# SeungheonOh/voxtral.c

Hardware: AMD Instinct MI355X
Metric: decoder tokens/sec + encoder RTF, Voxtral-4B bf16 at 1/2/4/8 MI355X (higher is better)
Workload: dtype f32

## Files before the change

include/voxtral_hip.h:

```cpp
#ifndef VOXTRAL_HIP_H
#define VOXTRAL_HIP_H

#include <stddef.h>
#include <stdint.h>

#ifdef __cplusplus
extern "C" {
#endif

int vox_hip_init(void);
int vox_hip_available(void);
void vox_hip_shutdown(void);
size_t vox_hip_memory_used(void);
const char *vox_hip_last_error(void);
void vox_hip_clear_error(void);
int vox_hip_set_device(int device);

typedef struct {
    int enc_dim, enc_layers, enc_heads, enc_kv_heads, enc_head_dim, enc_hidden, enc_window;
    int dec_dim, dec_layers, dec_heads, dec_kv_heads, dec_head_dim, dec_hidden, dec_window;
    int vocab, mel_bins, downsample, ada_dim;
    float rope_theta, enc_eps, dec_eps;
    int gelu_erf;
} vox_hip_config_t;

void vox_hip_config_voxtral_4b(vox_hip_config_t *cfg);

typedef struct {
    const float *conv0_w, *conv0_b, *conv1_w, *conv1_b;
    const uint16_t **enc_wq, **enc_wk, **enc_wv, **enc_wo, **enc_w1, **enc_w2, **enc_w3;
    const float **enc_wq_b, **enc_wv_b, **enc_wo_b, **enc_w2_b, **enc_attn_norm, **enc_ffn_norm;
    const float *enc_norm;
    const uint16_t *ad0, *ad1;
    const uint16_t *tok_emb;
    const uint16_t **dec_wq, **dec_wk, **dec_wv, **dec_wo, **dec_w1, **dec_w2, **dec_w3;
    const float **dec_attn_norm, **dec_ffn_norm, **dec_ada_down, **dec_ada_up;
    const float *dec_norm;
    const float **enc_wq_s, **enc_wk_s, **enc_wv_s, **enc_wo_s, **enc_w1_s, **enc_w2_s, **enc_w3_s;
    const float *ad0_s, *ad1_s, *tok_emb_s;
    const float **dec_wq_s, **dec_wk_s, **dec_wv_s, **dec_wo_s, **dec_w1_s, **dec_w2_s, **dec_w3_s;
} vox_hip_weights_t;

typedef struct vox_hip_model vox_hip_model_t;
typedef struct vox_hip_stream vox_hip_stream_t;

vox_hip_model_t *vox_hip_model_create(const vox_hip_config_t *cfg, const vox_hip_weights_t *w,
                                      int delay_tokens);
void vox_hip_model_free(vox_hip_model_t *m);
int vox_hip_model_set_delay(vox_hip_model_t *m, int delay_tokens);
int vox_hip_model_ada_scale(vox_hip_model_t *m, float *out);
int vox_hip_model_set_kv_fp16(vox_hip_model_t *m, int on);
int vox_hip_set_gemm_planes(int planes);
int vox_hip_gemm_planes(void);
int vox_hip_set_gemmf_wait(int ticks);

vox_hip_stream_t *vox_hip_stream_create(vox_hip_model_t *m);
void vox_hip_stream_free(vox_hip_stream_t *s);
int vox_hip_stream_kv_fp16(const vox_hip_stream_t *s);
int vox_hip_stream_reset(vox_hip_stream_t *s);
int vox_hip_stream_reset_decoder(vox_hip_stream_t *s);

int vox_hip_stream_encode_mel(vox_hip_stream_t *s, const float *mel, int n_frames,
                              int mel_on_device);
int vox_hip_stream_adapter_tokens(vox_hip_stream_t *s);
int vox_hip_stream_set_async_encode(vox_hip_stream_t *s, int on);
int vox_hip_stream_encode_mel_batch(vox_hip_stream_t *const *streams, const float *const *mels,
                                    const int *n_frames, int B, int mel_on_device, int *added);

typedef struct vox_hip_mel vox_hip_mel_t;
vox_hip_mel_t *vox_hip_mel_create(vox_hip_stream_t *s, int left_pad_samples);
int vox_hip_mel_feed(vox_hip_mel_t *m, const float *samples, int n_samples);
int vox_hip_mel_finish(vox_hip_mel_t *m, int right_pad_samples);
int vox_hip_mel_frames(const vox_hip_mel_t *m, int *frame_offset);
const float *vox_hip_mel_frame_ptr(const vox_hip_mel_t *m, int global_frame);
int vox_hip_mel_discard_before(vox_hip_mel_t *m, int keep_from_frame);
int vox_hip_mel_read(vox_hip_mel_t *m, int global_first, int n, float *out);
void vox_hip_mel_free(vox_hip_mel_t *m);
int vox_hip_mel_reset(vox_hip_mel_t *m, int left_pad_samples);
int vox_hip_stream_read_adapter(vox_hip_stream_t *s, int first, int n, float *out);

int vox_hip_stream_decode(vox_hip_stream_t *s, int max_steps, int stop_at_eos,
                          int *tokens_out, float *logits_out);
#define VOX_HIP_MAX_ALT 4
int vox_hip_stream_set_alt(vox_hip_stream_t *s, int n_alt, float cutoff);
int vox_hip_stream_read_alts(vox_hip_stream_t *s, int first, int n, int *ids_out, float *probs_out);
typedef struct vox_hip_batch vox_hip_batch_t;
vox_hip_batch_t *vox_hip_batch_create(vox_hip_model_t *m, int max_streams);
void vox_hip_batch_free(vox_hip_batch_t *b);
int vox_hip_batch_decode(vox_hip_batch_t *b, vox_hip_stream_t **streams, int n, int max_steps,
                         int stop_at_eos, int *tokens_out, int *counts_out);
int vox_hip_batch_decode_rows(vox_hip_batch_t *b, vox_hip_stream_t **streams, int n, const int *rows,
                              int max_steps, int stop_at_eos, int *tokens_out, int *counts_out);
int vox_hip_batch_begin_rows(vox_hip_batch_t *b, vox_hip_stream_t **streams, int n, const int *rows,
                             int max_steps, int stop_at_eos, int *tokens_out, int *counts_out);
int vox_hip_batch_finish(vox_hip_batch_t *b);
int vox_hip_batch_read_logits(vox_hip_batch_t *b, vox_hip_stream_t *s, float *out);
int vox_hip_batch_stats(const vox_hip_batch_t *b, long long *out6);
int vox_hip_stream_state(vox_hip_stream_t *s, int *out6);

void vox_hip_sgemm_bf16(int M, int N, int K, const float *A, const uint16_t *B_bf16, float *C);
void vox_hip_sgemm_q8(int M, int N, int K, const float *A, const int8_t *B_q8, const float *scales,
                      float *C);
void vox_hip_fused_qkv_bf16(int M, int K, const float *input,
                            const uint16_t *wq_bf16, int Nq, const uint16_t *wk_bf16, int Nk,
                            const uint16_t *wv_bf16, int Nv, float *q, float *k, float *v);
void vox_hip_fused_ffn_bf16(int M, int dim, int hidden, const float *input,
                            const uint16_t *w1_bf16, const uint16_t *w3_bf16,
                            const uint16_t *w2_bf16, float *output);
void vox_hip_encoder_attention(float *out, const float *Q, const float *K, const float *V,
                               int seq_q, int seq_k, int n_heads, int n_kv_heads,
                               int head_dim, float scale, int window_size, int q_offset);
int vox_hip_encoder_full_step(vox_hip_stream_t *s, float *x, int new_len,
                              const float *rope_freqs, int logical_start);
int vox_hip_decoder_prefill_step(vox_hip_stream_t *s, float *x, int seq_len,
                                 const float *rope_freqs, int logical_start);
void vox_hip_decoder_start(vox_hip_stream_t *s, const float *x, int dim);
void vox_hip_decoder_end(vox_hip_stream_t *s);
int vox_hip_decoder_full_step(vox_hip_stream_t *s, const float *rope_freqs, int logical_pos,
                              float *logits);

int vox_hip_stream_set_profiling(vox_hip_stream_t *s, int enable);
int vox_hip_stream_profile(vox_hip_stream_t *s, double *out8);
int vox_hip_stream_sync(vox_hip_stream_t *s);

void *vox_hip_device_upload(const void *host, size_t bytes);
int vox_hip_device_free(void *dev);

#ifdef __cplusplus
}
#endif
#endif
```

voxtral.c_amd/csrc/vox_hip.hip:

```cpp
#include "../../include/voxtral_hip.h"
#include "vox_hip_internal.h"

#include <hip/hip_runtime.h>
#include <math.h>
#include <stdarg.h>
#include <stdio.h>
#include <stdlib.h>
#include <string.h>

#include <stddef.h>
#include <algorithm>
#include <atomic>
#include <mutex>
#include <string>
#include <unordered_map>
#include <vector>

using namespace vox;

#define TOKEN_BOS 1
#define TOKEN_EOS 2
#define TOKEN_STREAMING_PAD 32

static thread_local std::string g_err;
static int g_inited = 0;
static size_t g_mem_used = 0;

static int set_err(const char* fmt, ...) {
    char buf[512];
    va_list ap;
    va_start(ap, fmt);
    vsnprintf(buf, sizeof buf, fmt, ap);
    va_end(ap);
    g_err = buf;
    fprintf(stderr, "voxtral_hip: %s\n", buf);
    return -1;
}

#define CK(expr)                                                                          \
    do {                                                                                  \
        hipError_t e__ = (expr);                                                          \
        if (e__ != hipSuccess)                                                            \
            return set_err("%s failed at %s:%d: %s", #expr, __FILE__, __LINE__, hipGetErrorString(e__)); \
    } while (0)

template <class T>
static hipError_t dalloc(T** p, size_t n) {
    *p = nullptr;
    if (n == 0) n = 1;
    hipError_t e = hipMalloc((void**)p, n * sizeof(T));
    if (e == hipSuccess) {
        g_mem_used += n * sizeof(T);
        e = hipMemsetAsync(*p, 0, n * sizeof(T), nullptr);
        if (e == hipSuccess) e = hipStreamSynchronize(nullptr);
    }
    return e;
}
static hipError_t h2d(void* dst, const void* src, size_t bytes) {
    hipError_t e = hipMemcpyAsync(dst, src, bytes, hipMemcpyHostToDevice, nullptr);
    return e == hipSuccess ? hipStreamSynchronize(nullptr) : e;
}
template <class T>
static void dfree(T*& p) {
    if (p) hipFree((void*)p);
    p = nullptr;
}

extern "C" const char* vox_hip_last_error(void) { return g_err.c_str(); }
extern "C" void vox_hip_clear_error(void) { g_err.clear(); }

extern "C" int vox_hip_init(void) {
    int n = 0;
    if (hipGetDeviceCount(&n) != hipSuccess || n <= 0) {
        set_err("no HIP device");
        return 0;
    }
    g_inited = 1;
    return 1;
}
extern "C" int vox_hip_available(void) { return g_inited; }
extern "C" void vox_hip_shutdown(void) { g_inited = 0; }
extern "C" size_t vox_hip_memory_used(void) { return g_mem_used; }
extern "C" int vox_hip_set_device(int device) {
    CK(hipSetDevice(device));
    return 0;
}

extern "C" void vox_hip_config_voxtral_4b(vox_hip_config_t* c) {
    c->enc_dim = 1280; c->enc_layers = 32; c->enc_heads = 32; c->enc_kv_heads = 32;
    c->enc_head_dim = 64; c->enc_hidden = 5120; c->enc_window = 750;
    c->dec_dim = 3072; c->dec_layers = 26; c->dec_heads = 32; c->dec_kv_heads = 8;
    c->dec_head_dim = 128; c->dec_hidden = 9216; c->dec_window = 8192;
    c->vocab = 131072; c->mel_bins = 128; c->downsample = 4; c->ada_dim = 32;
    c->rope_theta = 1000000.0f; c->enc_eps = 1e-5f; c->dec_eps = 1e-5f; c->gelu_erf = 0;
}

static float host_gelu(float v, int erf_mode) {
    if (erf_mode) return 0.5f * v * (1.0f + erff(v * 0.70710678118654752f));
    float x3 = v * v * v;
    float inner = 0.7978845608028654f * (v + 0.044715f * x3);
    return 0.5f * v * (1.0f + tanhf(inner));
}

static void host_rope(float* out, int p0, int n, int dim, float theta) {
    int half = dim / 2;
    for (int s = 0; s < n; s++) {
        float p = (float)(p0 + s);
        for (int d = 0; d < half; d++) {
            float freq = 1.0f / powf(theta, (float)(2 * d) / (float)dim);
            float ang = p * freq;
            out[(size_t)s * dim + 2 * d] = cosf(ang);
            out[(size_t)s * dim + 2 * d + 1] = sinf(ang);
        }
    }
}

struct EncLayerD {
    uint8_t *wqkv, *wo, *w13, *w2;
    float *sqkv, *so, *s13, *s2;
    float *bqkv, *bo, *b2, *attn_norm, *ffn_norm;
};
struct DecLayerD {
    uint8_t *wqkv, *wo, *w13, *w2;
    float *sqkv, *so, *s13, *s2;
    float *attn_norm, *ffn_norm;
};
struct DecFragD {
    uint8_t *wqkv, *wo, *w13, *w2;
};
static int frag_copy(uint8_t** dst, const uint8_t* src, int N, int K, int q8);
struct vox_hip_model;
static int model_frag(vox_hip_model* m);

struct vox_hip_model {
    vox_hip_config_t c;
    int delay_tokens;
    uint16_t *conv0_w, *conv1_w;
    float *conv0_b, *conv1_b, *enc_norm, *dec_norm;
    std::vector<EncLayerD> enc;
    std::vector<DecLayerD> dec;
    uint8_t *ad0, *ad1, *tok_emb;
    float *ad0_s, *ad1_s, *tok_emb_s;
    float* ada_scale;
    std::vector<float> ada_host;
    std::vector<std::vector<float>> ada_down, ada_up;
    float *rope_enc, *rope_dec;
    int rope_positions;
    int rope_gen;
    std::vector<DecFragD> dfrag;
    std::vector<DecFragD> efrag;
    uint8_t* lm_frag;
    int kv16;
};

static int upload(void* dst, const void* src, size_t bytes) {
    if (!src) return set_err("null weight pointer");
    CK(h2d(dst, src, bytes));
    return 0;
}

static int upload_f32_as_bf16(uint16_t* dst, const float* src, size_t n) {
    std::vector<uint16_t> tmp(n);
    for (size_t i = 0; i < n; i++) {
        uint32_t u;
        memcpy(&u, &src[i], 4);
        if (u & 0xffffu) return set_err("conv weight is not bf16-representable (element %zu)", i);
        tmp[i] = (uint16_t)(u >> 16);
    }
    return upload(dst, tmp.data(), n * 2);
}

static int upload_mat(uint8_t** dst, float** dscale, const void* src, const float* scale, size_t rows,
                      size_t cols) {
    const size_t esz = scale ? 1 : 2;
    CK(dalloc(dst, rows * cols * esz));
    if (upload(*dst, src, rows * cols * esz)) return -1;
    *dscale = nullptr;
    if (scale) {
        CK(dalloc(dscale, rows));
        if (upload(*dscale, scale, rows * 4)) return -1;
    }
    return 0;
}

static int upload_qkv(uint8_t** dst, float** dscale, const void* wq, const float* sq, const void* wk,
                      const float* sk, const void* wv, const float* sv, int nq, int nkv, int K) {
    if (!sq != !sk || !sq != !sv) return set_err("wq/wk/wv mix bf16 and Q8");
    const size_t esz = sq ? 1 : 2, rows = (size_t)nq + 2 * nkv;
    CK(dalloc(dst, rows * K * esz));
    if (upload(*dst, wq, (size_t)nq * K * esz) || upload(*dst + (size_t)nq * K * esz, wk, (size_t)nkv * K * esz) ||
        upload(*dst + (size_t)(nq + nkv) * K * esz, wv, (size_t)nkv * K * esz))
        return -1;
    *dscale = nullptr;
    if (sq) {
        CK(dalloc(dscale, rows));
        if (upload(*dscale, sq, (size_t)nq * 4) || upload(*dscale + nq, sk, (size_t)nkv * 4) ||
            upload(*dscale + nq + nkv, sv, (size_t)nkv * 4))
            return -1;
    }
    return 0;
}

static int upload_w13(uint8_t** dst, float** dscale, const void* w1, const float* s1, const void* w3,
                      const float* s3, int hidden, int K) {
    if (!w1 || !w3) return set_err("null w1/w3");
    if (!s1 != !s3) return set_err("w1/w3 mix bf16 and Q8");
    if (hidden % 16) return set_err("hidden %d not a multiple of 16", hidden);
    const size_t esz = s1 ? 1 : 2;
    CK(dalloc(dst, (size_t)2 * hidden * K * esz));
    size_t grp = (size_t)16 * K * esz;
    CK(hipMemcpy2D(*dst, 2 * grp, w1, grp, grp, hidden / 16, hipMemcpyHostToDevice));
    CK(hipMemcpy2D(*dst + grp, 2 * grp, w3, grp, grp, hidden / 16, hipMemcpyHostToDevice));
    *dscale = nullptr;
    if (s1) {
        CK(dalloc(dscale, (size_t)2 * hidden));
        const size_t g4 = 16 * 4;
        CK(hipMemcpy2D(*dscale, 2 * g4, s1, g4, g4, hidden / 16, hipMemcpyHostToDevice));
        CK(hipMemcpy2D((char*)*dscale + g4, 2 * g4, s3, g4, g4, hidden / 16, hipMemcpyHostToDevice));
    }
    return 0;
}

static int model_update_ada(vox_hip_model_t* m) {
    const vox_hip_config_t& c = m->c;
    int D = c.dec_dim, A = c.ada_dim;
    std::vector<float> t_cond(D), hidden(A);
    int half = D / 2;
    float log_theta = logf(10000.0f);
    float t = (float)m->delay_tokens;
    for (int i = 0; i < half; i++) {
        float inv_freq = expf(-log_theta * (float)i / (float)half);
        float emb = t * inv_freq;
        t_cond[i] = cosf(emb);
        t_cond[i + half] = sinf(emb);
    }
    m->ada_host.assign((size_t)c.dec_layers * D, 0.f);
    for (int l = 0; l < c.dec_layers; l++) {
        const float* down = m->ada_down[l].data();
        const float* up = m->ada_up[l].data();
        for (int i = 0; i < A; i++) {
            float sum = 0.f;
            for (int j = 0; j < D; j++) sum += down[(size_t)i * D + j] * t_cond[j];
            hidden[i] = host_gelu(sum, c.gelu_erf);
        }
        float* sc = m->ada_host.data() + (size_t)l * D;
        for (int i = 0; i < D; i++) {
            float sum = 0.f;
            for (int j = 0; j < A; j++) sum += up[(size_t)i * A + j] * hidden[j];
            sc[i] = sum;
        }
    }
    CK(h2d(m->ada_scale, m->ada_host.data(), m->ada_host.size() * 4));
    return 0;
}

static int model_rope_tables(vox_hip_model_t* m, int positions) {
    const vox_hip_config_t& c = m->c;
    dfree(m->rope_enc);
    dfree(m->rope_dec);
    std::vector<float> t((size_t)positions * std::max(c.enc_head_dim, c.dec_head_dim));
    CK(dalloc(&m->rope_enc, (size_t)positions * c.enc_head_dim));
    host_rope(t.data(), 0, positions, c.enc_head_dim, c.rope_theta);
    CK(h2d(m->rope_enc, t.data(), (size_t)positions * c.enc_head_dim * 4));
    CK(dalloc(&m->rope_dec, (size_t)positions * c.dec_head_dim));
    host_rope(t.data(), 0, positions, c.dec_head_dim, c.rope_theta);
    CK(h2d(m->rope_dec, t.data(), (size_t)positions * c.dec_head_dim * 4));
    m->rope_positions = positions;
    m->rope_gen++;
    return 0;
}

static int check_config(const vox_hip_config_t* c) {
    if (c->enc_head_dim != 64 && c->enc_head_dim != 128) return set_err("enc_head_dim must be 64/128");
    if (c->dec_head_dim != 64 && c->dec_head_dim != 128) return set_err("dec_head_dim must be 64/128");
    if (c->enc_heads % c->enc_kv_heads || c->dec_heads % c->dec_kv_heads)
        return set_err("heads must be a multiple of kv heads");
    if (c->dec_heads / c->dec_kv_heads > 4 || c->enc_heads / c->enc_kv_heads > 4)
        return set_err("GQA ratio > 4 unsupported");
    int dims[] = {c->enc_dim, c->enc_hidden, c->dec_dim, c->dec_hidden,
                  c->enc_heads * c->enc_head_dim, c->dec_heads * c->dec_head_dim,
                  c->dec_kv_heads * c->dec_head_dim, c->mel_bins * 3};
    for (int d : dims)
        if (d % 64) return set_err("dimension %d not a multiple of 64", d);
    if (c->vocab % 2) return set_err("vocab must be even");
    if (c->downsample != 4) return set_err("downsample must be 4");
    return 0;
}

extern "C" void vox_hip_model_free(vox_hip_model_t* m);

extern "C" vox_hip_model_t* vox_hip_model_create(const vox_hip_config_t* cfg,
                                                 const vox_hip_weights_t* w, int delay_tokens) {
    if (!g_inited && !vox_hip_init()) return nullptr;
    if (check_config(cfg)) return nullptr;
    vox_hip_model_t* m = new vox_hip_model_t();
    memset(&m->c, 0, sizeof m->c);
    m->c = *cfg;
    m->delay_tokens = delay_tokens;
    {
        const char* e = getenv("VOX_DECODER_KV_FP16");
        m->kv16 = (e && atoi(e) != 0 && cfg->dec_head_dim == 128) ? 1 : 0;
    }
    m->conv0_w = m->conv1_w = nullptr;
    m->ad0 = m->ad1 = m->tok_emb = nullptr;
    m->ad0_s = m->ad1_s = m->tok_emb_s = nullptr;
    m->conv0_b = m->conv1_b = m->enc_norm = m->dec_norm = m->ada_scale = nullptr;
    m->rope_enc = m->rope_dec = nullptr;
    const vox_hip_config_t& c = *cfg;
    const int ED = c.enc_dim, EQ = c.enc_heads * c.enc_head_dim, EKV = c.enc_kv_heads * c.enc_head_dim;
    const int EH = c.enc_hidden;
    const int DD = c.dec_dim, DQ = c.dec_heads * c.dec_head_dim, DKV = c.dec_kv_heads * c.dec_head_dim;
    const int DH = c.dec_hidden;
    auto fail = [&]() -> vox_hip_model_t* { vox_hip_model_free(m); return nullptr; };
#define TRY(x) do { if ((x) != 0) return fail(); } while (0)
#define TRYH(x) do { hipError_t e__ = (x); if (e__ != hipSuccess) { set_err("%s: %s", #x, hipGetErrorString(e__)); return fail(); } } while (0)
#define SCL(field, l) (w->field ? w->field[l] : nullptr)
    TRYH(dalloc(&m->conv0_w, (size_t)ED * c.mel_bins * 3));
    TRY(upload_f32_as_bf16(m->conv0_w, w->conv0_w, (size_t)ED * c.mel_bins * 3));
    TRYH(dalloc(&m->conv1_w, (size_t)ED * ED * 3));
    TRY(upload_f32_as_bf16(m->conv1_w, w->conv1_w, (size_t)ED * ED * 3));
    TRYH(dalloc(&m->conv0_b, ED));
    TRY(upload(m->conv0_b, w->conv0_b, ED * 4));
    TRYH(dalloc(&m->conv1_b, ED));
    TRY(upload(m->conv1_b, w->conv1_b, ED * 4));
    m->enc.resize(c.enc_layers);
    for (int l = 0; l < c.enc_layers; l++) {
        EncLayerD& L = m->enc[l];
        memset(&L, 0, sizeof L);
        TRY(upload_qkv(&L.wqkv, &L.sqkv, w->enc_wq[l], SCL(enc_wq_s, l), w->enc_wk[l], SCL(enc_wk_s, l),
                       w->enc_wv[l], SCL(enc_wv_s, l), EQ, EKV, ED));
        TRYH(dalloc(&L.bqkv, EQ + 2 * EKV));
        TRY(upload(L.bqkv, w->enc_wq_b[l], EQ * 4));
        TRY(upload(L.bqkv + EQ + EKV, w->enc_wv_b[l], EKV * 4));
        TRY(upload_mat(&L.wo, &L.so, w->enc_wo[l], SCL(enc_wo_s, l), ED, EQ));
        TRYH(dalloc(&L.bo, ED));
        TRY(upload(L.bo, w->enc_wo_b[l], ED * 4));
        TRY(upload_w13(&L.w13, &L.s13, w->enc_w1[l], SCL(enc_w1_s, l), w->enc_w3[l], SCL(enc_w3_s, l), EH, ED));
        TRY(upload_mat(&L.w2, &L.s2, w->enc_w2[l], SCL(enc_w2_s, l), ED, EH));
        TRYH(dalloc(&L.b2, ED));
        TRY(upload(L.b2, w->enc_w2_b[l], ED * 4));
        TRYH(dalloc(&L.attn_norm, ED));
        TRY(upload(L.attn_norm, w->enc_attn_norm[l], ED * 4));
        TRYH(dalloc(&L.ffn_norm, ED));
        TRY(upload(L.ffn_norm, w->enc_ffn_norm[l], ED * 4));
    }
    TRYH(dalloc(&m->enc_norm, ED));
    TRY(upload(m->enc_norm, w->enc_norm, ED * 4));
    TRY(upload_mat(&m->ad0, &m->ad0_s, w->ad0, w->ad0_s, DD, (size_t)ED * c.downsample));
    TRY(upload_mat(&m->ad1, &m->ad1_s, w->ad1, w->ad1_s, DD, DD));
    TRY(upload_mat(&m->tok_emb, &m->tok_emb_s, w->tok_emb, w->tok_emb_s, c.vocab, DD));
    m->dec.resize(c.dec_layers);
    m->ada_down.resize(c.dec_layers);
    m->ada_up.resize(c.dec_layers);
    for (int l = 0; l < c.dec_layers; l++) {
        DecLayerD& L = m->dec[l];
        memset(&L, 0, sizeof L);
        TRY(upload_qkv(&L.wqkv, &L.sqkv, w->dec_wq[l], SCL(dec_wq_s, l), w->dec_wk[l], SCL(dec_wk_s, l),
                       w->dec_wv[l], SCL(dec_wv_s, l), DQ, DKV, DD));
        TRY(upload_mat(&L.wo, &L.so, w->dec_wo[l], SCL(dec_wo_s, l), DD, DQ));
        TRY(upload_w13(&L.w13, &L.s13, w->dec_w1[l], SCL(dec_w1_s, l), w->dec_w3[l], SCL(dec_w3_s, l), DH, DD));
        TRY(upload_mat(&L.w2, &L.s2, w->dec_w2[l], SCL(dec_w2_s, l), DD, DH));
        TRYH(dalloc(&L.attn_norm, DD));
        TRY(upload(L.attn_norm, w->dec_attn_norm[l], DD * 4));
        TRYH(dalloc(&L.ffn_norm, DD));
        TRY(upload(L.ffn_norm, w->dec_ffn_norm[l], DD * 4));
        if (!w->dec_ada_down[l] || !w->dec_ada_up[l]) { set_err("null ada weights"); return fail(); }
        m->ada_down[l].assign(w->dec_ada_down[l], w->dec_ada_down[l] + (size_t)c.ada_dim * DD);
        m->ada_up[l].assign(w->dec_ada_up[l], w->dec_ada_up[l] + (size_t)DD * c.ada_dim);
    }
    TRYH(dalloc(&m->dec_norm, DD));
    TRY(upload(m->dec_norm, w->dec_norm, DD * 4));
    TRYH(dalloc(&m->ada_scale, (size_t)c.dec_layers * DD));
    TRY(model_update_ada(m));
    TRY(model_rope_tables(m, 32768));
#undef TRY
#undef TRYH
#undef SCL
    return m;
}

extern "C" void vox_hip_model_free(vox_hip_model_t* m) {
    if (!m) return;
    dfree(m->conv0_w); dfree(m->conv1_w); dfree(m->conv0_b); dfree(m->conv1_b);
    for (auto& L : m->enc) {
        dfree(L.wqkv); dfree(L.wo); dfree(L.w13); dfree(L.w2);
        dfree(L.sqkv); dfree(L.so); dfree(L.s13); dfree(L.s2);
        dfree(L.bqkv); dfree(L.bo); dfree(L.b2); dfree(L.attn_norm); dfree(L.ffn_norm);
    }
    for (auto& L : m->dec) {
        dfree(L.wqkv); dfree(L.wo); dfree(L.w13); dfree(L.w2);
        dfree(L.sqkv); dfree(L.so); dfree(L.s13); dfree(L.s2);
        dfree(L.attn_norm); dfree(L.ffn_norm);
    }
    for (auto& F : m->dfrag) {
        dfree(F.wqkv); dfree(F.wo); dfree(F.w13); dfree(F.w2);
    }
    for (auto& F : m->efrag) {
        dfree(F.wqkv); dfree(F.wo); dfree(F.w13); dfree(F.w2);
    }
    dfree(m->lm_frag);
    dfree(m->enc_norm); dfree(m->ad0); dfree(m->ad1); dfree(m->tok_emb); dfree(m->dec_norm);
    dfree(m->ad0_s); dfree(m->ad1_s); dfree(m->tok_emb_s);
    dfree(m->ada_scale); dfree(m->rope_enc); dfree(m->rope_dec);
    delete m;
}

extern "C" int vox_hip_model_set_delay(vox_hip_model_t* m, int delay_tokens) {
    m->delay_tokens = delay_tokens;
    return model_update_ada(m);
}

extern "C" int vox_hip_set_gemm_planes(int planes) {
    if (set_gemm_planes(planes)) return set_err("gemm planes: 2 or 3 (got %d)", planes);
    return 0;
}

extern "C" int vox_hip_gemm_planes(void) { return gemm_planes_np(); }
extern "C" int vox_hip_set_gemmf_wait(int ticks) { return set_gemmf_wait(ticks); }

extern "C" int vox_hip_model_set_kv_fp16(vox_hip_model_t* m, int on) {
    if (on && m->c.dec_head_dim != 128) return set_err("16-bit decoder KV: head_dim 128 only (got %d)", m->c.dec_head_dim);
    m->kv16 = on ? 1 : 0;
    return 0;
}

extern "C" int vox_hip_stream_kv_fp16(const vox_hip_stream_t* s);

extern "C" int vox_hip_model_ada_scale(vox_hip_model_t* m, float* out) {
    memcpy(out, m->ada_host.data(), m->ada_host.size() * 4);
    return 0;
}

static const int ENC_SUB = 1024;
static const int DEC_SLACK = 64;
static const int STEP_BATCH = 16;
static const size_t GEMM_WS_ELEMS = (size_t)8 << 20;
static const int TOKENS_CAP = 1 << 16;

struct vox_hip_stream {
    vox_hip_stream() { memset((void*)this, 0, offsetof(vox_hip_stream, pev)); }
    vox_hip_model_t* m;
    unsigned long long uid;
    hipStream_t st;
    float *ek, *ev, *dk, *dv;
    int ecap, dcap;
    int kv16;
    long long enc_pos;
    float *mel_p, *mel_tail, *c0_p, *c0_tail, *c0_res, *im2col;
    int res_count;
    int frames_cap;
    float *x_enc, *xn, *qkv, *q, *att, *gate, *enc_res;
    int x_rows_cap;
    int enc_res_count;
    float *rope_rows;
    int rope_rows_cap;
    float *adapter, *ad_mid;
    int adapter_cap, total_adapter;
    float *xd, *xnd, *qkvd, *qd_, *attd, *gated, *part, *logits, *pval;
    float *part_alt, *alts;
    float* gws;
    size_t gws_n;
    uint16_t* exp_;
    float* eslab;
    uint16_t* exp2;
    int* eticket;
    int enc_async;
    float* xbatch;
    float *cs_im, *cs_c0;
    float *abatch, *abatch_out;
    float* essq;
    uint16_t *gpa, *gpc;
    int* gflags;
    int gepoch;
    uint16_t *dpa, *dpc;
    int dp_rows;
    int n_alt;
    float alt_cutoff;
    int graph_alt;
    int graph_rope_gen;
    int *pidx, *state, *tokens;
    int* twin_state;
    int dec_rows_cap, tokens_cap;
    hipGraphExec_t step_exec[STEP_GRAPHS];
    int graph_ready;
    int started, eos_seen, n_generated;
    int h_state[4];
    int profiling;
    int graph_prof;
    int capturing;
    hipEvent_t evt[2];
    hipEvent_t sev;
    std::vector<hipEvent_t> pev;
    double prof_ms, prof_bytes;
    long long prof_launches;
};

static int stream_alloc_frames(vox_hip_stream_t* s, int frames) {
    if (frames <= s->frames_cap) return 0;
    const vox_hip_config_t& c = s->m->c;
    int f = 256;
    while (f < frames) f *= 2;
    dfree(s->mel_p); dfree(s->c0_p); dfree(s->im2col); dfree(s->x_enc);
    CK(dalloc(&s->mel_p, (size_t)(f + 2) * c.mel_bins));
    CK(dalloc(&s->c0_p, (size_t)(f + 3) * c.enc_dim));
    size_t im = std::max((size_t)f * c.mel_bins * 3, (size_t)(f / 2 + 2) * c.enc_dim * 3);
    CK(dalloc(&s->im2col, im));
    CK(dalloc(&s->x_enc, (size_t)(f / 2 + 8) * c.enc_dim));
    s->frames_cap = f;
    return 0;
}

static int stream_alloc_adapter(vox_hip_stream_t* s, int need) {
    if (need <= s->adapter_cap) return 0;
    const int D = s->m->c.dec_dim;
    int nc = s->adapter_cap ? s->adapter_cap : 1024;
    while (nc < need) nc *= 2;
    float* na = nullptr;
    CK(dalloc(&na, (size_t)nc * D));
    if (s->adapter && s->total_adapter > 0)
        CK(hipMemcpyAsync(na, s->adapter, (size_t)s->total_adapter * D * 4, hipMemcpyDeviceToDevice, s->st));
    CK(hipStreamSynchronize(s->st));
    dfree(s->adapter);
    s->adapter = na;
    s->adapter_cap = nc;
    s->graph_ready = 0;
    return 0;
}

static int stream_alloc_dec_rows(vox_hip_stream_t* s, int rows) {
    if (rows <= s->dec_rows_cap) return 0;
    const vox_hip_config_t& c = s->m->c;
    int r = 64;
    while (r < rows) r *= 2;
    const int DQ = c.dec_heads * c.dec_head_dim, DKV = c.dec_kv_heads * c.dec_head_dim;
    dfree(s->xd); dfree(s->xnd); dfree(s->qkvd); dfree(s->qd_); dfree(s->attd); dfree(s->gated);
    CK(dalloc(&s->xd, (size_t)r * c.dec_dim));
    CK(dalloc(&s->xnd, (size_t)r * c.dec_dim));
    CK(dalloc(&s->qkvd, (size_t)r * (DQ + 2 * DKV)));
    CK(dalloc(&s->qd_, (size_t)r * DQ));
    CK(dalloc(&s->attd, (size_t)r * DQ));
    CK(dalloc(&s->gated, (size_t)r * c.dec_hidden));
    s->dec_rows_cap = r;
    s->graph_ready = 0;
    return 0;
}

extern "C" void vox_hip_stream_free(vox_hip_stream_t* s);

extern "C" vox_hip_stream_t* vox_hip_stream_create(vox_hip_model_t* m) {
    static std::atomic<unsigned long long> next_uid{1};
    vox_hip_stream_t* s = new vox_hip_stream_t();
    s->m = m;
    s->uid = next_uid++;
    const vox_hip_config_t& c = m->c;
    auto fail = [&]() -> vox_hip_stream_t* { vox_hip_stream_free(s); return nullptr; };
#define TRYH(x) do { hipError_t e__ = (x); if (e__ != hipSuccess) { set_err("%s: %s", #x, hipGetErrorString(e__)); return fail(); } } while (0)
#define SCL(field, l) (w->field ? w->field[l] : nullptr)
// ... 1017 lines not shown
    }
    if (!s->enc_async) CK(hipStreamSynchronize(s->st));
    return added;
}

extern "C" int vox_hip_stream_set_async_encode(vox_hip_stream_t* s, int on) {
    if (!s) return set_err("null stream");
    if (s->enc_async && !on) CK(hipStreamSynchronize(s->st));
    s->enc_async = on ? 1 : 0;
    return 0;
}

extern "C" int vox_hip_stream_adapter_tokens(vox_hip_stream_t* s) { return s->total_adapter; }

extern "C" int vox_hip_stream_read_adapter(vox_hip_stream_t* s, int first, int n, float* out) {
    const int D = s->m->c.dec_dim;
    if (first < 0 || first + n > s->total_adapter) return set_err("adapter rows out of range");
    CK(hipMemcpyAsync(out, s->adapter + (size_t)first * D, (size_t)n * D * 4, hipMemcpyDeviceToHost, s->st));
    CK(hipStreamSynchronize(s->st));
    return 0;
}

static int stream_prefilled(vox_hip_stream_t* s, hipStream_t q) {
    const int np = 32 + s->m->delay_tokens;
    const int st4[4] = {np, np, TOKEN_STREAMING_PAD, s->n_generated};
    CK(hipMemcpyAsync(s->state, st4, sizeof st4, hipMemcpyHostToDevice, q));
    s->h_state[0] = np;
    s->h_state[1] = np;
    s->h_state[2] = TOKEN_STREAMING_PAD;
    s->h_state[3] = s->n_generated;
    s->started = 1;
    return 0;
}

static int dec_gemmf_env() {
    static int v = -1;
    if (v < 0) {
        const char* e = getenv("VOX_HIP_PREFILL_GEMMF");
        v = (e && atoi(e) == 0) ? 0 : 1;
    }
    return v;
}

static bool dec_gemmf_ok(const vox_hip_model_t* m, int n) {
    const vox_hip_config_t& c = m->c;
    const int DD = c.dec_dim, DQ = c.dec_heads * c.dec_head_dim, DKV = c.dec_kv_heads * c.dec_head_dim;
    return enc_gemmf_env() && dec_gemmf_env() && !m->dec[0].sqkv && n >= 1 && n <= PLANE_MAX_ROWS && gemmf_ok(n, DQ + 2 * DKV, DD) &&
           gemmf_ok(n, DD, DQ) && gemmf_ok(n, 2 * c.dec_hidden, DD) && gemmf_ok(n, DD, c.dec_hidden) &&
           c.dec_hidden % 64 == 0;
}

static int stream_dec_planes(vox_hip_stream_t* s, int rows) {
    if (rows <= s->dp_rows) return 0;
    const vox_hip_config_t& c = s->m->c;
    const int DD = c.dec_dim, DQ = c.dec_heads * c.dec_head_dim;
    const int r = (rows + 127) / 128 * 128;
    dfree(s->dpa);
    dfree(s->dpc);
    s->dp_rows = 0;
    CK(dalloc(&s->dpa, (size_t)r * 3 * std::max(DD, DQ)));
    CK(dalloc(&s->dpc, (size_t)r * 3 * c.dec_hidden));
    if (!s->gflags) CK(dalloc(&s->gflags, gemmf_flag_ints()));
    s->dp_rows = r;
    return 0;
}

template <class Attn>
static int dec_layers_gemmf(vox_hip_stream_t* s, const GemmfQ& q, float* x, int n, Attn attn) {
    vox_hip_model_t* m = s->m;
    const vox_hip_config_t& c = m->c;
    const int DD = c.dec_dim, DQ = c.dec_heads * c.dec_head_dim, DKV = c.dec_kv_heads * c.dec_head_dim;
    const int DH = c.dec_hidden;
    if (model_frag(m) || stream_dec_planes(s, n)) return -1;
    for (int l = 0; l < c.dec_layers; l++) {
        const DecLayerD& L = m->dec[l];
        const DecFragD& F = m->dfrag[l];
        CK(launch_rmsnorm_fplanes(x, n, DD, L.attn_norm, nullptr, c.dec_eps, s->dpa, nullptr, 0, q.st));
        if (gemmf_on(q, EPI_STORE, s->dpa, DD, n, F.wqkv, DQ + 2 * DKV, nullptr, s->qkvd, DQ + 2 * DKV, nullptr)) return -1;
        if (attn(l)) return -1;
        if (gemmf_on(q, EPI_RESID, s->dpa, DQ, n, F.wo, DD, nullptr, x, DD, nullptr)) return -1;
        CK(launch_rmsnorm_fplanes(x, n, DD, L.ffn_norm, m->ada_scale + (size_t)l * DD, c.dec_eps, s->dpa, nullptr, 0,
                                  q.st));
        if (gemmf_on(q, EPI_SWIGLU, s->dpa, DD, n, F.w13, 2 * DH, nullptr, nullptr, DH, s->dpc)) return -1;
        if (gemmf_on(q, EPI_RESID, s->dpc, DH, n, F.w2, DD, nullptr, x, DD, nullptr)) return -1;
    }
    return 0;
}

static int run_decoder_rows(vox_hip_stream_t* s, float* x, int n, int pos0, const float* rope) {
    vox_hip_model_t* m = s->m;
    const vox_hip_config_t& c = m->c;
    const int DD = c.dec_dim, H = c.dec_heads, KVH = c.dec_kv_heads, hd = c.dec_head_dim;
    const int DQ = H * hd, DKV = KVH * hd, DH = c.dec_hidden;
    const float scale = 1.0f / sqrtf((float)hd);
    hipStream_t st = s->st;
    if (stream_alloc_dec_rows(s, n)) return -1;
    if (n > DEC_SLACK + 1 && pos0 > 0) return set_err("prefill of %d rows on a non-empty cache", n);
    bool gf = n > 1 && dec_gemmf_ok(m, n);
    if (gf && (model_frag(m) || stream_dec_planes(s, n))) {
        vox_hip_clear_error();
        (void)hipGetLastError();
        gf = false;
    }
    if (gf) {
        if (!s->gflags) CK(dalloc(&s->gflags, gemmf_flag_ints()));
        return dec_layers_gemmf(s, GemmfQ{st, s->gws, s->gws_n, s->gflags, &s->gepoch}, x, n, [&](int l) -> int {
            float* Kc = dec_ring(s, s->dk, l);
            float* Vc = dec_ring(s, s->dv, l);
            CK(launch_rope_kv(s->qkvd, n, DQ, DKV, hd, rope, pos0, s->qd_, Kc, Vc, s->dcap, st, s->kv16));
            CK(launch_attn_rows_mf(hd, s->qd_, DQ, Kc, Vc, s->dcap, s->attd, DQ, n, H, KVH, pos0, 0, c.dec_window, scale,
                                   st, s->gws, s->gws_n, s->dpa, s->kv16));
            return 0;
        });
    }
    for (int l = 0; l < c.dec_layers; l++) {
        const DecLayerD& L = m->dec[l];
        float* Kc = dec_ring(s, s->dk, l);
        float* Vc = dec_ring(s, s->dv, l);
        CK(launch_rmsnorm_rows(x, DD, s->xnd, DD, L.attn_norm, nullptr, n, DD, c.dec_eps, st));
        CK(launch_gemm(EPI_STORE, 3, s->xnd, DD, L.wqkv, L.sqkv, DD, n, DQ + 2 * DKV, nullptr, s->qkvd, DQ + 2 * DKV, st, s->gws, s->gws_n));
        CK(launch_rope_kv(s->qkvd, n, DQ, DKV, hd, rope, pos0, s->qd_, Kc, Vc, s->dcap, st, s->kv16));
        CK(launch_attn_rows_mf(hd, s->qd_, DQ, Kc, Vc, s->dcap, s->attd, DQ, n, H, KVH, pos0, 0, c.dec_window, scale, st,
                             s->gws, s->gws_n, nullptr, s->kv16));
        CK(launch_gemm(EPI_RESID, 3, s->attd, DQ, L.wo, L.so, DQ, n, DD, nullptr, x, DD, st, s->gws, s->gws_n));
        CK(launch_rmsnorm_rows(x, DD, s->xnd, DD, L.ffn_norm, m->ada_scale + (size_t)l * DD, n, DD, c.dec_eps, st));
        CK(launch_gemm(EPI_SWIGLU, 3, s->xnd, DD, L.w13, L.s13, DD, n, 2 * DH, nullptr, s->gated, DH, st, s->gws, s->gws_n));
        CK(launch_gemm(EPI_RESID, 3, s->gated, DH, L.w2, L.s2, DH, n, DD, nullptr, x, DD, st, s->gws, s->gws_n));
    }
    return 0;
}

static int enqueue_lm_head(vox_hip_stream_t* s, const int* state);

static int enqueue_step_layers(vox_hip_stream_t* s, const int* state, int pos, const float* rope_row,
                               int splits) {
    vox_hip_model_t* m = s->m;
    const vox_hip_config_t& c = m->c;
    const int DD = c.dec_dim, H = c.dec_heads, KVH = c.dec_kv_heads, hd = c.dec_head_dim;
    const int DQ = H * hd, DKV = KVH * hd, DH = c.dec_hidden;
    const float scale = 1.0f / sqrtf((float)hd);
    hipStream_t st = s->st;
    for (int l = 0; l < c.dec_layers; l++) {
        const DecLayerD& L = m->dec[l];
        float* Kc = dec_ring(s, s->dk, l);
        float* Vc = dec_ring(s, s->dv, l);
        GemvArgs a;
        memset(&a, 0, sizeof a);
        a.x = s->xd; a.K = DD; a.W = L.wqkv; a.wscale = L.sqkv; a.rows = DQ + 2 * DKV;
        a.norm_w = L.attn_norm; a.eps = c.dec_eps; a.y = s->qd_;
        a.qd = DQ; a.kvd = DKV; a.hd = hd;
        a.state = state; a.pos = pos;
        a.rope = state ? m->rope_dec : rope_row - (size_t)pos * hd;
        a.Kc = Kc; a.Vc = Vc; a.cap = s->dcap; a.kv16 = s->kv16;
        CK(launch_gemv(PRO_NORM, EPI_QKV, a, st));
        CK(launch_attn_decode(hd, s->qd_, Kc, Vc, s->dcap, state, pos, c.dec_window, scale, H, KVH,
                              s->part, s->attd, splits, st, s->kv16));
        memset(&a, 0, sizeof a);
        a.x = s->attd; a.K = DQ; a.W = L.wo; a.wscale = L.so; a.rows = DD; a.y = s->xd;
        CK(launch_gemv(PRO_NONE, EPI_RESID, a, st));
        memset(&a, 0, sizeof a);
        a.x = s->xd; a.K = DD; a.W = L.w13; a.wscale = L.s13; a.rows = 2 * DH; a.norm_w = L.ffn_norm;
        a.ada = m->ada_scale + (size_t)l * DD; a.eps = c.dec_eps; a.y = s->gated;
        const bool gprof = s->profiling && state && !s->capturing && (int)s->pev.size() == 2 * c.dec_layers;
        if (gprof) CK(launch_gemv_timed(PRO_NORM_ADA, EPI_SWIGLU, a, s->pev[2 * l], s->pev[2 * l + 1], st));
        else CK(launch_gemv(PRO_NORM_ADA, EPI_SWIGLU, a, st));
        memset(&a, 0, sizeof a);
        a.x = s->gated; a.K = DH; a.W = L.w2; a.wscale = L.s2; a.rows = DD; a.y = s->xd;
        CK(launch_gemv(PRO_NONE, EPI_RESID, a, st));
    }
    return enqueue_lm_head(s, state);
}

static int enqueue_lm_head(vox_hip_stream_t* s, const int* state) {
    vox_hip_model_t* m = s->m;
    const vox_hip_config_t& c = m->c;
    hipStream_t st = s->st;
    GemvArgs a;
    memset(&a, 0, sizeof a);
    a.x = s->xd; a.K = c.dec_dim; a.W = m->tok_emb; a.wscale = m->tok_emb_s; a.rows = c.vocab; a.norm_w = m->dec_norm;
    a.eps = c.dec_eps; a.y = s->logits; a.part_val = s->pval; a.part_idx = s->pidx;
    a.part_alt = s->part_alt;
    CK(launch_gemv(PRO_NORM, (state && s->n_alt > 1) ? EPI_LOGITS_ALT : EPI_LOGITS, a, st));
    return 0;
}

static int graph_splits(const vox_hip_stream_t* s, int g) {
    return std::min(1 << g, attn_maxsplits(s->m->c.dec_window));
}

static int graph_index(const vox_hip_stream_t* s, int ctx) {
    const int need = (ctx + ATT_BLOCK_KEYS - 1) / ATT_BLOCK_KEYS;
    int g = 0;
    while ((1 << g) < need && (1 << g) < attn_maxsplits(s->m->c.dec_window)) g++;
    return g;
}

static int enqueue_graph_step(vox_hip_stream_t* s, int splits) {
    const vox_hip_config_t& c = s->m->c;
    if (enqueue_step_layers(s, s->state, 0, nullptr, splits)) return -1;
    CK(launch_argmax_final(s->pval, s->pidx, gemv_grid(c.vocab), s->state, s->tokens, s->tokens_cap,
                           s->adapter, s->adapter_cap, s->m->tok_emb, s->m->tok_emb_s, c.dec_dim, s->xd,
                           s->part_alt, s->n_alt > 1 ? s->alts : nullptr, s->st));
    return 0;
}

static int build_step_graph(vox_hip_stream_t* s, int gi) {
    if (s->step_exec[gi]) {
        hipGraphExecDestroy(s->step_exec[gi]);
        s->step_exec[gi] = nullptr;
    }
    hipGraph_t g = nullptr;
    CK(hipStreamBeginCapture(s->st, hipStreamCaptureModeThreadLocal));
    s->capturing = 1;
    int rc = enqueue_graph_step(s, graph_splits(s, gi));
    s->capturing = 0;
    hipError_t e = hipStreamEndCapture(s->st, &g);
    if (rc || e != hipSuccess) {
        if (g) hipGraphDestroy(g);
        return set_err("graph capture failed: %s", hipGetErrorString(e));
    }
    e = hipGraphInstantiate(&s->step_exec[gi], g, nullptr, nullptr, 0);
    hipGraphDestroy(g);
    if (e != hipSuccess) return set_err("graph instantiate failed: %s", hipGetErrorString(e));
    s->graph_ready |= 1 << gi;
    s->graph_alt = s->n_alt > 1;
    s->graph_rope_gen = s->m->rope_gen;
    return 0;
}

static int collect_graph_profile(vox_hip_stream_t* s) {
    if (!s->profiling || !s->graph_prof) return 0;
    const vox_hip_config_t& c = s->m->c;
    for (int l = 0; l < c.dec_layers; l++) {
        float ms = 0.f;
        CK(hipEventElapsedTime(&ms, s->pev[2 * l], s->pev[2 * l + 1]));
        s->prof_ms += ms;
        s->prof_bytes += (double)2 * c.dec_hidden * c.dec_dim * 2;
        s->prof_launches++;
    }
    return 0;
}

static int use_graphs() {
    static int v = -1;
    if (v < 0) {
        const char* e = getenv("VOX_HIP_GRAPH");
        v = (e && atoi(e) == 0) ? 0 : 1;
    }
    return v;
}

static int run_steps(vox_hip_stream_t* s, int n, int pos0) {
    const vox_hip_config_t& c = s->m->c;
    const int gi = graph_index(s, std::min(pos0 + n, c.dec_window));
    const int splits = graph_splits(s, gi);
    if (s->profiling && use_graphs() && n > 1) {
        s->profiling = 0;
        const int rc = run_steps(s, n - 1, pos0);
        s->profiling = 1;
        if (rc) return -1;
        pos0 += n - 1;
        n = 1;
    }
    if (!use_graphs() || s->profiling) {
        if (s->profiling && s->pev.empty()) {
            s->pev.resize(2 * c.dec_layers);
            for (auto& e : s->pev) CK(hipEventCreate(&e));
        }
        s->graph_prof = s->profiling;
        for (int i = 0; i < n; i++)
            if (enqueue_graph_step(s, splits)) return -1;
        return 0;
    }
    if (s->graph_ready && (s->graph_alt != (s->n_alt > 1) || s->graph_rope_gen != s->m->rope_gen)) s->graph_ready = 0;
    if (!(s->graph_ready & (1 << gi)) && build_step_graph(s, gi)) return -1;
    for (int i = 0; i < n; i++) CK(hipGraphLaunch(s->step_exec[gi], s->st));
    return 0;
}

template <class T>
static int ring_read(const T* ring, int cap, int rec, long long first, int n, T* out, hipStream_t st) {
    while (n > 0) {
        const int slot = (int)(first % cap);
        const int k = std::min(n, cap - slot);
        CK(hipMemcpyAsync(out, ring + (size_t)slot * rec, (size_t)k * rec * sizeof(T), hipMemcpyDeviceToHost, st));
        out += (size_t)k * rec;
        first += k;
        n -= k;
    }
    return 0;
}

static int stream_prefill(vox_hip_stream_t* s) {
    vox_hip_model_t* m = s->m;
    const int np = 32 + m->delay_tokens;
    if (stream_alloc_dec_rows(s, np)) return -1;
    if (ensure_rope(s, np + 2)) return -1;
    CK(launch_embed_rows(s->adapter, m->tok_emb, m->tok_emb_s, 0, np, TOKEN_BOS, TOKEN_STREAMING_PAD, m->c.dec_dim,
                         s->xd, s->st));
    if (run_decoder_rows(s, s->xd, np, 0, m->rope_dec)) return -1;
    return stream_prefilled(s, s->st);
}

extern "C" int vox_hip_stream_decode(vox_hip_stream_t* s, int max_steps, int stop_at_eos,
                                     int* tokens_out, float* logits_out) {
    vox_hip_model_t* m = s->m;
    const vox_hip_config_t& c = m->c;
    const int D = c.dec_dim, V = c.vocab, hd = c.dec_head_dim;
    const int prompt_len = 1 + 32 + m->delay_tokens;
    int produced = 0;
    if (max_steps <= 0 || s->eos_seen) return 0;
    if (!s->started) {
        if (s->total_adapter < prompt_len) return 0;
        if (stream_prefill(s)) return -1;
    }
    const int step_base = s->n_generated;
    int avail = s->total_adapter - (s->h_state[1] > 0 ? s->h_state[1] : prompt_len - 1);
    {
        int st4[4];
        CK(hipMemcpyAsync(st4, s->state, sizeof st4, hipMemcpyDeviceToHost, s->st));
        CK(hipStreamSynchronize(s->st));
        memcpy(s->h_state, st4, sizeof st4);
        avail = s->total_adapter - st4[1];
    }
    if (ensure_rope(s, (long long)s->h_state[0] + avail + 1)) return -1;
    if (avail > 0) CK(launch_embed_step(s->adapter, m->tok_emb, m->tok_emb_s, s->state, D, s->xd, s->st));
    int todo = std::min(max_steps, avail);
    std::vector<int> tok;
    while (produced < todo) {
        int b = std::min(STEP_BATCH, todo - produced);
        if (logits_out) b = 1;
        if (run_steps(s, b, s->h_state[0] + produced)) return -1;
        tok.resize(produced + b);
        if (ring_read(s->tokens, s->tokens_cap, 1, (long long)step_base + produced, b, tok.data() + produced, s->st))
// ... 69 lines not shown
            if (pr) pr[k] = p;
        }
    }
    return 0;
}

extern "C" int vox_hip_stream_state(vox_hip_stream_t* s, int* out6) {
    out6[0] = s->h_state[0];
    out6[1] = s->h_state[1];
    out6[2] = s->h_state[2];
    out6[3] = s->started;
    out6[4] = s->eos_seen;
    out6[5] = s->n_generated;
    return 0;
}

extern "C" int vox_hip_stream_set_profiling(vox_hip_stream_t* s, int enable) {
    s->profiling = enable;
    s->prof_ms = 0;
    s->prof_bytes = 0;
    s->prof_launches = 0;
    return 0;
}

extern "C" int vox_hip_stream_profile(vox_hip_stream_t* s, double* out8) {
    out8[0] = s->prof_ms;
    out8[1] = s->prof_bytes;
    out8[2] = (double)s->prof_launches;
    out8[3] = s->prof_launches ? s->prof_ms / s->prof_launches : 0.0;
    out8[4] = 0;
    out8[5] = s->prof_launches ? s->prof_bytes / s->prof_launches : 0.0;
    int rec = 0;
    if (s->gflags) {
        CK(hipMemcpyAsync(&rec, s->gflags + gemmf_grid(), sizeof rec, hipMemcpyDeviceToHost, s->st));
        CK(hipStreamSynchronize(s->st));
    }
    out8[6] = rec;
    out8[7] = 0.0;
    return 0;
}

struct TwinW {
    uint8_t* w;
    float* s;
    int N, K, Np, Kp;
};
struct TwinKey {
    const void* p;
    int n, k;
    bool operator==(const TwinKey& o) const { return p == o.p && n == o.n && k == o.k; }
};
struct TwinKeyHash {
    size_t operator()(const TwinKey& t) const {
        return std::hash<const void*>()(t.p) ^ ((size_t)t.n * 0x9e3779b97f4a7c15ull) ^ ((size_t)t.k << 1);
    }
};
static std::mutex g_twin_mu;
static std::unordered_map<TwinKey, TwinW, TwinKeyHash> g_wcache;
static hipStream_t g_twin_st = nullptr;
static float* g_twin_ws = nullptr;
static float *g_tA = nullptr, *g_tC = nullptr, *g_tQ = nullptr, *g_tK = nullptr, *g_tV = nullptr, *g_tO = nullptr;
static size_t g_tA_n = 0, g_tC_n = 0, g_tQ_n = 0, g_tK_n = 0, g_tV_n = 0, g_tO_n = 0;
static float* g_tWs = nullptr;
static size_t g_tWs_n = 0;

static int pad_to(int v, int a) { return (v + a - 1) / a * a; }

static int twin_buf(float** p, size_t* cap, size_t n) {
    if (n <= *cap) return 0;
    dfree(*p);
    *cap = 0;
    CK(dalloc(p, n));
    *cap = n;
    return 0;
}

static const TwinW* twin_weight(const void* host, const float* scales, int N, int K) {
    if (!host || N <= 0 || K <= 0) {
        set_err("twin weight: null pointer or empty shape (%d x %d)", N, K);
        return nullptr;
    }
    const TwinKey key{host, N, K};
    auto it = g_wcache.find(key);
    if (it != g_wcache.end()) return &it->second;
    TwinW t{nullptr, nullptr, N, K, pad_to(N, 128), pad_to(K, 64)};
    const size_t esz = scales ? 1 : 2;
    hipError_t e = dalloc(&t.w, (size_t)t.Np * t.Kp * esz);
    if (e == hipSuccess)
        e = hipMemcpy2DAsync(t.w, (size_t)t.Kp * esz, host, (size_t)K * esz, (size_t)K * esz, N,
                             hipMemcpyHostToDevice, g_twin_st);
    if (e == hipSuccess && scales) {
        e = dalloc(&t.s, (size_t)t.Np);
        if (e == hipSuccess) e = hipMemcpyAsync(t.s, scales, (size_t)N * 4, hipMemcpyHostToDevice, g_twin_st);
    }
    if (e == hipSuccess) e = hipStreamSynchronize(g_twin_st);
    if (e != hipSuccess) {
        dfree(t.w);
        dfree(t.s);
        set_err("twin weight upload (%d x %d): %s", N, K, hipGetErrorString(e));
        return nullptr;
    }
    return &(g_wcache[key] = t);
}

static int twin_init() {
    if (!g_inited && !vox_hip_init()) return -1;
    if (!g_twin_st) CK(hipStreamCreateWithFlags(&g_twin_st, hipStreamNonBlocking));
    if (!g_twin_ws) CK(dalloc(&g_twin_ws, GEMM_WS_ELEMS));
    return 0;
}

static int twin_put_rows(float** buf, size_t* cap, const float* host, int M, int K, int Kp) {
    if (!host) return set_err("twin: null input");
    if (twin_buf(buf, cap, (size_t)M * Kp)) return -1;
    if (Kp != K) {
        CK(hipMemsetAsync(*buf, 0, (size_t)M * Kp * 4, g_twin_st));
        CK(hipMemcpy2DAsync(*buf, (size_t)Kp * 4, host, (size_t)K * 4, (size_t)K * 4, M, hipMemcpyHostToDevice,
                            g_twin_st));
    } else {
        CK(hipMemcpyAsync(*buf, host, (size_t)M * K * 4, hipMemcpyHostToDevice, g_twin_st));
    }
    return 0;
}

static int twin_get_rows(float* host, const float* dev, int M, int N, int Np) {
    if (!host) return set_err("twin: null output");
    CK(hipMemcpy2DAsync(host, (size_t)N * 4, dev, (size_t)Np * 4, (size_t)N * 4, M, hipMemcpyDeviceToHost, g_twin_st));
    return 0;
}

static int twin_gemm_dev(int M, const float* dA, const TwinW& W, float* dC) {
    if (M == 1 && gemv_ok(W.Np, W.Kp, W.s != nullptr)) {
        GemvArgs a;
        memset(&a, 0, sizeof a);
        a.x = dA; a.K = W.Kp; a.W = W.w; a.wscale = W.s; a.rows = W.Np; a.y = dC;
        CK(launch_gemv(PRO_NONE, EPI_STORE, a, g_twin_st));
        return 0;
    }
    CK(launch_gemm(EPI_STORE, 3, dA, W.Kp, W.w, W.s, W.Kp, M, W.Np, nullptr, dC, W.Np, g_twin_st, g_twin_ws,
                   GEMM_WS_ELEMS));
    return 0;
}

static int twin_sgemm(int M, int N, int K, const float* A, const void* B, const float* scales, float* C) {
    if (M <= 0 || N <= 0 || K <= 0) return M == 0 ? 0 : set_err("sgemm: bad shape %d x %d x %d", M, N, K);
    if (twin_init()) return -1;
    const TwinW* W = twin_weight(B, scales, N, K);
    if (!W) return -1;
    if (twin_put_rows(&g_tA, &g_tA_n, A, M, K, W->Kp) || twin_buf(&g_tC, &g_tC_n, (size_t)M * W->Np) ||
        twin_gemm_dev(M, g_tA, *W, g_tC) || twin_get_rows(C, g_tC, M, N, W->Np))
        return -1;
    CK(hipStreamSynchronize(g_twin_st));
    return 0;
}

extern "C" void vox_hip_sgemm_bf16(int M, int N, int K, const float* A, const uint16_t* B, float* C) {
    std::lock_guard<std::mutex> lk(g_twin_mu);
    twin_sgemm(M, N, K, A, B, nullptr, C);
}

extern "C" void vox_hip_sgemm_q8(int M, int N, int K, const float* A, const int8_t* B, const float* scales,
                                 float* C) {
    std::lock_guard<std::mutex> lk(g_twin_mu);
    if (!scales) { set_err("sgemm_q8: null scales"); return; }
    twin_sgemm(M, N, K, A, B, scales, C);
}

extern "C" void vox_hip_fused_qkv_bf16(int M, int K, const float* input, const uint16_t* wq, int Nq,
                                       const uint16_t* wk, int Nk, const uint16_t* wv, int Nv,
                                       float* q, float* k, float* v) {
    std::lock_guard<std::mutex> lk(g_twin_mu);
    if (M <= 0) return;
    if (twin_init()) return;
    const TwinW* W[3] = {twin_weight(wq, nullptr, Nq, K), twin_weight(wk, nullptr, Nk, K),
                         twin_weight(wv, nullptr, Nv, K)};
    if (!W[0] || !W[1] || !W[2]) return;
    float* outs[3] = {q, k, v};
    float* dO[3] = {nullptr, nullptr, nullptr};
    size_t* caps[3] = {&g_tQ_n, &g_tK_n, &g_tV_n};
    float** bufs[3] = {&g_tQ, &g_tK, &g_tV};
    if (twin_put_rows(&g_tA, &g_tA_n, input, M, K, W[0]->Kp)) return;
    for (int i = 0; i < 3; i++) {
        if (twin_buf(bufs[i], caps[i], (size_t)M * W[i]->Np) || twin_gemm_dev(M, g_tA, *W[i], *bufs[i])) return;
        dO[i] = *bufs[i];
    }
    for (int i = 0; i < 3; i++)
        if (twin_get_rows(outs[i], dO[i], M, W[i]->N, W[i]->Np)) return;
    if (hipStreamSynchronize(g_twin_st) != hipSuccess) set_err("fused_qkv: sync failed");
}

__global__ void k_silu_mul(float* g, const float* u, size_t n) {
    size_t i = (size_t)blockIdx.x * 256 + threadIdx.x;
    if (i < n) {
        float v = g[i];
        g[i] = v / (1.0f + expf(-v)) * u[i];
    }
}

extern "C" void vox_hip_fused_ffn_bf16(int M, int dim, int hidden, const float* input,
                                       const uint16_t* w1, const uint16_t* w3, const uint16_t* w2,
                                       float* output) {
    std::lock_guard<std::mutex> lk(g_twin_mu);
    if (M <= 0) return;
    if (twin_init()) return;
    const TwinW* d1 = twin_weight(w1, nullptr, hidden, dim);
    const TwinW* d3 = twin_weight(w3, nullptr, hidden, dim);
    const TwinW* d2 = twin_weight(w2, nullptr, dim, hidden);
    if (!d1 || !d3 || !d2) return;
    const int Hp = d1->Np;
    if (d2->Kp != Hp) { set_err("fused_ffn: padded hidden %d != %d", d2->Kp, Hp); return; }
    if (twin_put_rows(&g_tA, &g_tA_n, input, M, dim, d1->Kp) || twin_buf(&g_tQ, &g_tQ_n, (size_t)M * Hp) ||
        twin_buf(&g_tK, &g_tK_n, (size_t)M * Hp) || twin_buf(&g_tC, &g_tC_n, (size_t)M * d2->Np) ||
        twin_gemm_dev(M, g_tA, *d1, g_tQ) || twin_gemm_dev(M, g_tA, *d3, g_tK))
        return;
    const size_t n = (size_t)M * Hp;
    hipLaunchKernelGGL(k_silu_mul, dim3((unsigned)((n + 255) / 256)), dim3(256), 0, g_twin_st, g_tQ, g_tK, n);
    if (hipGetLastError() != hipSuccess) { set_err("fused_ffn: silu_mul launch failed"); return; }
    if (twin_gemm_dev(M, g_tQ, *d2, g_tC) || twin_get_rows(output, g_tC, M, dim, d2->Np)) return;
    if (hipStreamSynchronize(g_twin_st) != hipSuccess) set_err("fused_ffn: sync failed");
}

static int twin_attention(float* out, const float* Q, const float* K, const float* V, int seq_q, int seq_k,
                          int n_heads, int n_kv_heads, int head_dim, float scale, int window_size, int q_offset) {
    if (twin_init()) return -1;
    if (seq_q <= 0) return 0;
    if (!out || !Q || !K || !V) return set_err("encoder_attention: null pointer");
    if (q_offset < 0 || q_offset + seq_q > seq_k) return set_err("encoder_attention: queries beyond keys");
    if (n_kv_heads <= 0 || n_heads % n_kv_heads) return set_err("encoder_attention: heads %d / kv heads %d", n_heads, n_kv_heads);
    const size_t qn = (size_t)seq_q * n_heads * head_dim, kn = (size_t)seq_k * n_kv_heads * head_dim;
    if (twin_buf(&g_tQ, &g_tQ_n, qn) || twin_buf(&g_tK, &g_tK_n, kn) || twin_buf(&g_tV, &g_tV_n, kn) ||
        twin_buf(&g_tO, &g_tO_n, qn))
        return -1;
    CK(hipMemcpyAsync(g_tQ, Q, qn * 4, hipMemcpyHostToDevice, g_twin_st));
    CK(hipMemcpyAsync(g_tK, K, kn * 4, hipMemcpyHostToDevice, g_twin_st));
    CK(hipMemcpyAsync(g_tV, V, kn * 4, hipMemcpyHostToDevice, g_twin_st));
    const int W = window_size > 0 ? window_size : (1 << 30);
    float* ws = nullptr;
    size_t wsn = 0;
    if (n_heads * ((seq_q + 15) / 16) < 256) {
        wsn = (size_t)n_heads * seq_q * 16 * (head_dim + 2);
        if (twin_buf(&g_tWs, &g_tWs_n, wsn)) return -1;
        ws = g_tWs;
    }
    CK(launch_attn_rows_mf(head_dim, g_tQ, n_heads * head_dim, g_tK, g_tV, seq_k, g_tO, n_heads * head_dim, seq_q,
                         n_heads, n_kv_heads, q_offset, 0, W, scale, g_twin_st, ws, wsn));
    CK(hipMemcpyAsync(out, g_tO, qn * 4, hipMemcpyDeviceToHost, g_twin_st));
    CK(hipStreamSynchronize(g_twin_st));
    return 0;
}

extern "C" void vox_hip_encoder_attention(float* out, const float* Q, const float* K, const float* V,
                                          int seq_q, int seq_k, int n_heads, int n_kv_heads,
                                          int head_dim, float scale, int window_size, int q_offset) {
    std::lock_guard<std::mutex> lk(g_twin_mu);
    twin_attention(out, Q, K, V, seq_q, seq_k, n_heads, n_kv_heads, head_dim, scale, window_size, q_offset);
}

static int upload_rope_rows(vox_hip_stream_t* s, const float* rope, size_t n) {
    if (n > (size_t)s->rope_rows_cap) {
        dfree(s->rope_rows);
        CK(dalloc(&s->rope_rows, n));
        s->rope_rows_cap = (int)n;
    }
    CK(hipMemcpyAsync(s->rope_rows, rope, n * 4, hipMemcpyHostToDevice, s->st));
    return 0;
}

extern "C" int vox_hip_encoder_full_step(vox_hip_stream_t* s, float* x, int new_len,
                                         const float* rope_freqs, int logical_start) {
    const vox_hip_config_t& c = s->m->c;
    const int ED = c.enc_dim;
    if (stream_alloc_frames(s, 2 * new_len + 8)) return -1;
    float* xin = s->x_enc + (size_t)4 * ED;
    CK(hipMemcpyAsync(xin, x, (size_t)new_len * ED * 4, hipMemcpyHostToDevice, s->st));
    if (upload_rope_rows(s, rope_freqs, (size_t)new_len * c.enc_head_dim)) return -1;
    for (int r0 = 0; r0 < new_len; r0 += ENC_SUB) {
        int nr = std::min(ENC_SUB, new_len - r0);
        if (run_encoder_rows(s, xin + (size_t)r0 * ED, nr, (long long)logical_start + r0,
                             s->rope_rows + (size_t)r0 * c.enc_head_dim))
            return -1;
    }
    CK(hipMemcpyAsync(x, xin, (size_t)new_len * ED * 4, hipMemcpyDeviceToHost, s->st));
    CK(hipStreamSynchronize(s->st));
    return 0;
}

extern "C" int vox_hip_decoder_prefill_step(vox_hip_stream_t* s, float* x, int seq_len,
                                            const float* rope_freqs, int logical_start) {
    const vox_hip_config_t& c = s->m->c;
    if (stream_alloc_dec_rows(s, seq_len)) return -1;
    CK(hipMemcpyAsync(s->xd, x, (size_t)seq_len * c.dec_dim * 4, hipMemcpyHostToDevice, s->st));
    if (upload_rope_rows(s, rope_freqs, (size_t)seq_len * c.dec_head_dim)) return -1;
    if (run_decoder_rows(s, s->xd, seq_len, logical_start, s->rope_rows)) return -1;
    CK(hipMemcpyAsync(x, s->xd, (size_t)seq_len * c.dec_dim * 4, hipMemcpyDeviceToHost, s->st));
    CK(hipStreamSynchronize(s->st));
    return 0;
}

extern "C" void vox_hip_decoder_start(vox_hip_stream_t* s, const float* x, int dim) {
    if (!s || !x || dim != s->m->c.dec_dim) {
        set_err("decoder_start: dim %d != dec_dim", dim);
        return;
    }
    if (hipMemcpyAsync(s->xd, x, (size_t)dim * 4, hipMemcpyHostToDevice, s->st) != hipSuccess)
        set_err("decoder_start upload failed");
}
// ... 590 lines not shown
```

voxtral.c_amd/csrc/vox_hip_dev.h:

```cpp
#pragma once
#include <hip/hip_runtime.h>
#include <stdint.h>

#include "vox_hip_internal.h"

namespace vox {

typedef __attribute__((ext_vector_type(8))) __bf16 bf16x8;
typedef __attribute__((ext_vector_type(4))) float f32x4;
typedef __attribute__((ext_vector_type(2))) float f32x2;
typedef __attribute__((ext_vector_type(4))) unsigned int u32x4;
typedef __attribute__((ext_vector_type(2))) unsigned int u32x2;

__device__ __forceinline__ uint4 ldnt(const uint4* p) {
    u32x4 v = __builtin_nontemporal_load(reinterpret_cast<const u32x4*>(p));
    return make_uint4(v.x, v.y, v.z, v.w);
}

__device__ __forceinline__ float bf2f(uint32_t bits16) { return __uint_as_float(bits16 << 16); }
__device__ __forceinline__ float bflo(uint32_t w) { return __uint_as_float(w << 16); }
__device__ __forceinline__ float bfhi(uint32_t w) { return __uint_as_float(w & 0xffff0000u); }

__device__ __forceinline__ uint32_t f2bf(float f) {
    const __bf16 b = (__bf16)f;
    return __builtin_bit_cast(unsigned short, b);
}

template <int CTRL>
__device__ __forceinline__ float dpp(float v) {
    return __int_as_float(__builtin_amdgcn_update_dpp(0, __float_as_int(v), CTRL, 0xF, 0xF, false));
}
__device__ __forceinline__ float rows4_sum(float v) {
    const int iv = __float_as_int(v);
    const float a = __int_as_float(__builtin_amdgcn_readlane(iv, 0)), b = __int_as_float(__builtin_amdgcn_readlane(iv, 16));
    const float c = __int_as_float(__builtin_amdgcn_readlane(iv, 32)), d = __int_as_float(__builtin_amdgcn_readlane(iv, 48));
    return (a + b) + (c + d);
}
__device__ __forceinline__ float rows4_max(float v) {
    const int iv = __float_as_int(v);
    const float a = __int_as_float(__builtin_amdgcn_readlane(iv, 0)), b = __int_as_float(__builtin_amdgcn_readlane(iv, 16));
    const float c = __int_as_float(__builtin_amdgcn_readlane(iv, 32)), d = __int_as_float(__builtin_amdgcn_readlane(iv, 48));
    return fmaxf(fmaxf(a, b), fmaxf(c, d));
}
__device__ __forceinline__ float row_sum16(float v) {
    v += dpp<0xB1>(v);
    v += dpp<0x4E>(v);
    v += dpp<0x141>(v);
    v += dpp<0x140>(v);
    return v;
}
__device__ __forceinline__ float row_max16(float v) {
    v = fmaxf(v, dpp<0xB1>(v));
    v = fmaxf(v, dpp<0x4E>(v));
    v = fmaxf(v, dpp<0x141>(v));
    v = fmaxf(v, dpp<0x140>(v));
    return v;
}
__device__ __forceinline__ float wave_sum(float v) {
    v = row_sum16(v);
    v += __shfl_xor(v, 16, 64);
    v += __shfl_xor(v, 32, 64);
    return v;
}
__device__ __forceinline__ float wave_sum63(float v) {
    v = row_sum16(v);
    v += __int_as_float(__builtin_amdgcn_update_dpp(0, __float_as_int(v), 0x142, 0xA, 0xF, false));
    v += __int_as_float(__builtin_amdgcn_update_dpp(0, __float_as_int(v), 0x143, 0xC, 0xF, false));
    return v;
}
__device__ __forceinline__ float wave_max(float v) {
    v = row_max16(v);
    v = fmaxf(v, __shfl_xor(v, 16, 64));
    v = fmaxf(v, __shfl_xor(v, 32, 64));
    return v;
}

__device__ __forceinline__ float gelu_tanh(float v) {
    float x3 = v * v * v;
    float inner = 0.7978845608028654f * (v + 0.044715f * x3);
    return 0.5f * v * (1.0f + tanhf(inner));
}
__device__ __forceinline__ float gelu_erf(float v) { return 0.5f * v * (1.0f + erff(v * 0.70710678118654752f)); }
__device__ __forceinline__ float silu(float v) { return v / (1.0f + expf(-v)); }

__device__ __forceinline__ void split3(float v, uint16_t& h, uint16_t& m, uint16_t& l) {
    const uint32_t b0 = f2bf(v);
    const float r1 = v - __uint_as_float(b0 << 16);
    const uint32_t b1 = f2bf(r1);
    const float r2 = r1 - __uint_as_float(b1 << 16);
    h = (uint16_t)b0;
    m = (uint16_t)b1;
    l = (uint16_t)f2bf(r2);
}

__device__ __forceinline__ size_t frag_off(int j, int k) {
    const int b = k >> 6, r = k & 63;
    return ((size_t)(b * 2 + ((r >> 3) & 1)) * 64 + (r >> 4) * 16 + j) * 8 + (r & 7);
}

__device__ __forceinline__ float psum(const float* __restrict__ part, int S, int N, int j, int n) {
    part += (size_t)(j >> 4) * S * SK_ROWS * N;
    j &= 15;
    float v = part[(size_t)j * N + n];
#pragma unroll 4
    for (int s = 1; s < S; s++) v += part[((size_t)s * SK_ROWS + j) * N + n];
    return v;
}
__device__ __forceinline__ float2 psum2(const float* __restrict__ part, int S, int N, int j, int n) {
    part += (size_t)(j >> 4) * S * SK_ROWS * N + (size_t)(j & 15) * N + n;
    const size_t stride = (size_t)SK_ROWS * N;
    float2 v = *reinterpret_cast<const float2*>(part);
    for (int s0 = 1; s0 < S; s0 += 8) {
        float2 t[8];
#pragma unroll
        for (int c = 0; c < 8; c++)
            t[c] = s0 + c < S ? *reinterpret_cast<const float2*>(part + (s0 + c) * stride) : make_float2(0.f, 0.f);
#pragma unroll
        for (int c = 0; c < 8; c++)
            if (s0 + c < S) {
                v.x += t[c].x;
                v.y += t[c].y;
            }
    }
    return v;
}
__device__ __forceinline__ size_t frag_at(int j, int K, int p, int k) {
    return ((size_t)(j >> 4) * 3 + p) * SK_ROWS * K + frag_off(j & 15, k);
}

__device__ __forceinline__ float dot8(uint4 w, float4 a, float4 b, float acc) {
    acc = fmaf(bflo(w.x), a.x, acc);
    acc = fmaf(bfhi(w.x), a.y, acc);
    acc = fmaf(bflo(w.y), a.z, acc);
    acc = fmaf(bfhi(w.y), a.w, acc);
    acc = fmaf(bflo(w.z), b.x, acc);
    acc = fmaf(bfhi(w.z), b.y, acc);
    acc = fmaf(bflo(w.w), b.z, acc);
    acc = fmaf(bfhi(w.w), b.w, acc);
    return acc;
}

__device__ __forceinline__ float i8f(uint32_t w, int b) { return (float)((int32_t)(w << (24 - 8 * b)) >> 24); }
__device__ __forceinline__ float dot16q(uint4 w, const float4 (&x)[4], float acc) {
    const uint32_t d[4] = {w.x, w.y, w.z, w.w};
#pragma unroll
    for (int k = 0; k < 4; k++) {
        acc = fmaf(i8f(d[k], 0), x[k].x, acc);
        acc = fmaf(i8f(d[k], 1), x[k].y, acc);
        acc = fmaf(i8f(d[k], 2), x[k].z, acc);
        acc = fmaf(i8f(d[k], 3), x[k].w, acc);
    }
    return acc;
}

}
```

voxtral.c_amd/csrc/vox_hip_internal.h:

```cpp
#pragma once
#include <hip/hip_runtime.h>
#include <stdint.h>

namespace vox {

enum { EPI_STORE = 0, EPI_RESID = 1, EPI_GELU = 2, EPI_GELU_ERF = 3, EPI_SWIGLU = 4, EPI_QKV = 5, EPI_LOGITS = 6,
       EPI_LOGITS_ALT = 7,
       EPI_PARTIAL = 8,
       EPI_QKV_BIAS = 9 };
constexpr int ALT_TEXT_MIN = 1000;
constexpr int ALT_PART = 10;
constexpr int ALT_REC = 8;
enum { PRO_NONE = 0, PRO_NORM = 1, PRO_NORM_ADA = 2 };

constexpr int GEMV_MAX_BLOCKS = 1024;

struct GemvArgs {
    const float* x;
    int K;
    const void* W;
    const float* wscale;
    int rows;
    const float* norm_w;
    const float* ada;
    float eps;
    float* y;
    const float* bias;
    int qd, kvd, hd;
    const float* rope;
    const int* state;
    int pos;
    float* Kc;
    float* Vc;
    int cap;
    int kv16 = 0;
    float* part_val;
    int* part_idx;
    float* part_alt;
};

constexpr int VOX_MAX_BATCH = 32;

struct BatchSlot {
    int* state;
    int* tokens;
    const float* adapter;
    char* Kc;
    char* Vc;
    float* alts;
    int adapter_rows;
    int left;
    int stop_tok;
    int live;
    int pos;
    int produced;
};
static_assert(sizeof(BatchSlot) == 72, "BatchSlot layout");
constexpr int BATCH_TOKLOG = 64;

struct AttnPtrs {
    const float* q[VOX_MAX_BATCH];
    const float* Kc[VOX_MAX_BATCH];
    const float* Vc[VOX_MAX_BATCH];
    const int* state[VOX_MAX_BATCH];
    float* part[VOX_MAX_BATCH];
    float* out[VOX_MAX_BATCH];
    const BatchSlot* slots = nullptr;
    size_t ring_off = 0;
};

struct AttnFuse {
    const float* qkv;
    int S, N;
    const float* rope;
    uint16_t* xs;
};

constexpr int ARGB = 64;

int gemv_grid(int rows);
bool gemv_ok(int rows, int K, int q8);
int attn_maxch(int window);
int attn_maxsplits(int window);
hipError_t launch_rmsnorm_rows(const float* x, int ldx, float* y, int ldy, const float* w,
                               const float* ada, int M, int D, float eps, hipStream_t st);
hipError_t launch_gemm(int epi, int nsplit, const float* A, int lda, const void* W,
                       const float* wscale, int K, int M, int N, const float* bias, float* C,
                       int ldc, hipStream_t st, float* ws = nullptr, size_t ws_elems = 0);
hipError_t launch_rope_kv(const float* qkv, int M, int qd, int kvd, int hd, const float* rope,
                          int pos0, float* q, float* Kc, float* Vc, int cap, hipStream_t st, int kv16 = 0);
hipError_t launch_attn_rows_mf(int hd, const float* Q, int ldq, const float* Kc, const float* Vc,
                             int cap, float* O, int ldo, int M, int H, int KVH, int q_pos0,
                             int k_first, int window, float scale, hipStream_t st, float* ws = nullptr,
                             size_t ws_elems = 0, uint16_t* xs = nullptr, int kv16 = 0);
hipError_t launch_slabs_rope_kv(const float* part, int S, int M, const float* bias, int qd, int kvd, int hd,
                                const float* rope, int pos0, float* q, float* Kc, float* Vc, int cap, hipStream_t st);
hipError_t launch_gemv(int pro, int epi, const GemvArgs& a, hipStream_t st);
const void* gemv_kernel(int pro, int epi, const GemvArgs& a);
hipError_t launch_gemv_timed(int pro, int epi, const GemvArgs& a, hipEvent_t start, hipEvent_t stop,
                             hipStream_t st);
int gemv_occupancy(const void* fn);
hipError_t launch_attn_decode(int hd, const float* q, const float* Kc, const float* Vc, int cap,
                              const int* state, int pos_host, int window, float scale, int H,
                              int KVH, float* part, float* out, int splits, hipStream_t st, int kv16 = 0);
hipError_t launch_attn_decode_batch(int hd, const AttnPtrs& p, int nb, int cap, int window, float scale,
                                    int H, int KVH, int splits, hipStream_t st, int kv16 = 0);
constexpr int ATT_BLOCK_KEYS = 256;
hipError_t launch_attn_batch_fused(int hd, const AttnPtrs& p, const AttnFuse& f, int nb, int cap, int window,
                                   float scale, int H, int KVH, int splits, hipStream_t st, int kv16 = 0);

struct EncRows {
    int B;
    int off[VOX_MAX_BATCH], nr[VOX_MAX_BATCH], pos0[VOX_MAX_BATCH];
    float* Kc[VOX_MAX_BATCH];
    float* Vc[VOX_MAX_BATCH];
};
hipError_t launch_rope_kv_rows(const float* qkv, int N, int qd, int kvd, int hd, const float* rope_table,
                               const EncRows& er, float* q, int cap, hipStream_t st);
hipError_t launch_attn_rows(int hd, const float* Q, const EncRows& er, int N, int cap, float* O, int H, int KVH,
                            int window, float scale, float* ws, size_t ws_elems, hipStream_t st, uint16_t* xs = nullptr);
constexpr int STEP_GRAPHS = 8;
hipError_t launch_attn_batch_dbg(const AttnPtrs& p, const AttnFuse& f, int nb, int cap, int window, float scale, int H,
                                 int KVH, int splits, hipStream_t st);
hipError_t launch_attn_dbg(int dbg, const float* q, const float* Kc, const float* Vc, int cap,
                           const int* state, float* part, float* out, hipStream_t st);
hipError_t launch_embed_step(const float* adapter, const void* emb, const float* esc, const int* state,
                             int D, float* x, hipStream_t st);
hipError_t launch_embed_rows(const float* adapter, const void* emb, const float* esc, int row0, int n,
                             int first_tok, int rest_tok, int D, float* x, hipStream_t st);
hipError_t launch_argmax_final(const float* pv, const int* pi, int n, int* state, int* tokens,
                               int cap, const float* adapter, int adapter_rows,
                               const void* emb, const float* esc, int D, float* x,
                               const float* part_alt, float* alts, hipStream_t st);
hipError_t launch_embed_batch(const BatchSlot* slots, int nb, const void* emb, const float* esc, int D, float* x,
                              hipStream_t st);
hipError_t launch_argmax_batch(const float* logits, int nb, int V, float* pval, int* pidx, float* palt,
                               BatchSlot* slots, int tokens_cap, int* toklog, const void* emb, const float* esc, int D,
                               float* x, hipStream_t st);
#ifdef VOX_KBENCH
#define VOX_KB_KNOB(name, v) int name = v
#else
#define VOX_KB_KNOB(name, v) constexpr int name = v
#endif
constexpr int SK_ROWS = 16;
constexpr int SK_MAX_ROWS = 96;
constexpr int PLANE_MAX_ROWS = 1024;
hipError_t launch_frag_pack(const void* src, int N, int K, int q8, void* dst, hipStream_t st);
hipError_t launch_rmsnorm_fplanes(float* x, int nb, int D, const float* w, const float* ada, float eps,
                                  uint16_t* xs, const float* part, int S, hipStream_t st, const float* bias = nullptr);
hipError_t launch_resid_slabs(float* x, int nb, int D, const float* part, int S, const float* bias, hipStream_t st);
hipError_t launch_slabs_rows(const float* part, int S, int nb, int N, const float* bias, float* out, int ldo,
                             hipStream_t st);
hipError_t launch_split_fplanes(const float* x, int nb, int K, uint16_t* xs, hipStream_t st);
hipError_t launch_swiglu_fplanes(const float* part, int S, int H, int nb, uint16_t* xs, hipStream_t st);
hipError_t launch_gemm_skf(const uint16_t* xs, int K, const void* Wf, const float* wscale, int N, int nb, float* C,
                           int ldc, hipStream_t st);
hipError_t launch_gemm_skf2(const uint16_t* xs, int K, const void* Wf, const float* wscale, int N, int nb, float* C,
                            int ldc, hipStream_t st);
int skl_splits(int K, int N = 0);
constexpr int SKL_MAX_SLICES = 12;
hipError_t launch_gemm_skl(const uint16_t* xs, int K, const void* Wf, const float* wscale, int N, int nb,
                           float* part, hipStream_t st, const float* ssq = nullptr, int nsl = 0, float eps = 0.f,
                           int pair = 0);
hipError_t launch_gemm_skl_cfg(int nw, int ks, const uint16_t* xs, int K, const void* Wf, int N, int nb, float* part,
                               hipStream_t st);
hipError_t launch_gemm_skl2_cfg(int nw, int ks, const uint16_t* xs, int K, const void* Wf, int N, int nb, float* part,
                                hipStream_t st);
hipError_t launch_resid_xw_fplanes(float* x, int nb, int D, const float* w, const float* ada, uint16_t* xs,
                                   const float* part, int S, const float* bias, float* ssq, hipStream_t st);
enum { SKX_PRO_PLANES = 0, SKX_PRO_SCALE = 1 };
enum { SKX_EPI_QKV = 1, SKX_EPI_RESID = 2, SKX_EPI_SWIGLU = 3 };
struct SklFused {
    const float* ssq_in = nullptr;
    int nsl = 0;
    float eps = 0.f;
    float* part = nullptr;
    int* ticket = nullptr;
    const float* bias = nullptr;
    float* x = nullptr;
    float* ssq_out = nullptr;
    uint16_t* planes = nullptr;
    const float* nw = nullptr;
    const float* ada = nullptr;
    const float* rope = nullptr;
    int qd = 0, kvd = 0, hd = 0, pos0 = 0, cap = 0;
    float* q = nullptr;
    float* Kc = nullptr;
    float* Vc = nullptr;
};
int sklx_slices(int N, int K);
constexpr int SKX_TICKETS = 4 * 1024;
hipError_t launch_gemm_sklx(int pro, int epi, const uint16_t* xs, int K, const void* Wf, int N, int nb,
                            const SklFused& f, hipStream_t st);
bool gemmf_ok(int M, int N, int K);
int gemmf_grid();
size_t gemmf_flag_ints();
int set_gemmf_wait(int ticks);
size_t gemmf_ws_floats(int blocks);
hipError_t launch_gemmf(int epi, int np, const uint16_t* xs, int K, int M, const void* Wf, int N, const float* bias,
                        float* C, int ldc, uint16_t* xo, float* ws, size_t ws_floats, int* flags, int epoch,
                        hipStream_t st);
int gemm_planes_np();
int set_gemm_planes(int np);
hipError_t launch_im2col3(const float* src, int C, int T, int stride, int off, float* A,
                          hipStream_t st);
hipError_t launch_mel_tail(const float* melp, int n_new, int MB, float* tail, hipStream_t st);
hipError_t launch_mel_frames(const float* samples, long long start0, int nframes, const float* window,
                             const float* dcosT, const float* dsinT, const float* filtT, float log_min, float* mel,
                             hipStream_t st);
hipError_t launch_mel_reflect(float* buf, long long n, long long real_end, int len, hipStream_t st);

}
```

voxtral.c_amd/csrc/vox_hip_kernels.hip:

```cpp
#include "vox_hip_internal.h"
#include "vox_hip_dev.h"

#include <hip/hip_runtime.h>
#include <hip/hip_ext.h>
#include <stdint.h>
#include <algorithm>
#include <string.h>
#include <stdlib.h>

namespace vox {

typedef _Float16 kvh_t;
typedef _Float16 h16x4 __attribute__((ext_vector_type(4)));
typedef _Float16 h16x2 __attribute__((ext_vector_type(2)));
template <class T> __device__ __forceinline__ float4 kv_ld4(const T* p) {
    if constexpr (sizeof(T) == 4) {
        return *reinterpret_cast<const float4*>(p);
    } else {
        const h16x4 h = *reinterpret_cast<const h16x4*>(p);
        return make_float4((float)h[0], (float)h[1], (float)h[2], (float)h[3]);
    }
}
template <class T> __device__ __forceinline__ float2 kv_ld2(const T* p) {
    if constexpr (sizeof(T) == 4) {
// ... 453 lines not shown
                for (int b = 0; b < NB; b++) vv[c][b] = vn[c][b];
        }
    }
    if (g == 0) {
        sm[wave][j] = m;
        sl[wave][j] = l;
    }
#pragma unroll
    for (int i = 0; i < 4; i++)
#pragma unroll
        for (int b = 0; b < NB; b++) so[wave][4 * g + i][NB * j + b] = acc[b][i];
    __syncthreads();
    const int r = tid >> 4, d0 = (tid & 15) * NB;
    if (r >= nq) return;
    float mx = -1e30f;
#pragma unroll
    for (int w = 0; w < 4; w++) mx = fmaxf(mx, sm[w][r]);
    float f[4], den = 0.f;
#pragma unroll
    for (int w = 0; w < 4; w++) {
        f[w] = expf(sm[w][r] - mx);
        den = fmaf(f[w], sl[w][r], den);
    }
    float num[NB];
#pragma unroll
    for (int e = 0; e < NB; e++) {
        num[e] = 0.f;
#pragma unroll
        for (int w = 0; w < 4; w++) num[e] = fmaf(f[w], so[w][r][d0 + e], num[e]);
    }
    if (ns > 1) {
        float* pp = part + ((size_t)(h * M + rbase + q0 + r) * ns + zsplit) * (HD + 2);
#pragma unroll
        for (int e = 0; e < NB; e++) pp[d0 + e] = num[e];
        if ((tid & 15) == 0) {
            pp[HD] = mx;
            pp[HD + 1] = den;
        }
    } else if (xs) {
        const float inv = den > 0.f ? 1.0f / den : 0.f;
        const int row = rbase + q0 + r, K = H * HD;
#pragma unroll
        for (int e0 = 0; e0 < NB; e0 += 4) {
            uint16_t hh[4], mm[4], ll[4];
#pragma unroll
            for (int e = 0; e < 4; e++) split3(num[e0 + e] * inv, hh[e], mm[e], ll[e]);
            const int k = h * HD + d0 + e0;
            *reinterpret_cast<uint2*>(xs + frag_at(row, K, 0, k)) = make_uint2(hh[0] | ((uint32_t)hh[1] << 16), hh[2] | ((uint32_t)hh[3] << 16));
            *reinterpret_cast<uint2*>(xs + frag_at(row, K, 1, k)) = make_uint2(mm[0] | ((uint32_t)mm[1] << 16), mm[2] | ((uint32_t)mm[3] << 16));
            *reinterpret_cast<uint2*>(xs + frag_at(row, K, 2, k)) = make_uint2(ll[0] | ((uint32_t)ll[1] << 16), ll[2] | ((uint32_t)ll[3] << 16));
        }
    } else {
        const float inv = den > 0.f ? 1.0f / den : 0.f;
        float* op = O + (size_t)(rbase + q0 + r) * ldo + h * HD + d0;
#pragma unroll
        for (int e = 0; e < NB; e++) op[e] = num[e] * inv;
    }
}

template <int HD>
__global__ __launch_bounds__(HD) void k_attn_tiled_combine(const float* __restrict__ part, int ns, int M,
                                                           float* __restrict__ O, int ldo, uint16_t* __restrict__ xs) {
    __shared__ __attribute__((aligned(16))) float sv[HD];
    const int h = blockIdx.x, q = blockIdx.y, d = threadIdx.x;
    const float* pp = part + (size_t)(h * M + q) * ns * (HD + 2);
    float mx = -1e30f, num = 0.f, den = 0.f;
    for (int z0 = 0; z0 < ns; z0 += 8) {
        float zm[8], zl[8], zv[8];
#pragma unroll
        for (int c = 0; c < 8; c++) {
            const float* pz = pp + (size_t)min(z0 + c, ns - 1) * (HD + 2);
            zm[c] = pz[HD];
            zl[c] = pz[HD + 1];
            zv[c] = pz[d];
        }
        float cm = mx;
#pragma unroll
        for (int c = 0; c < 8; c++)
            if (z0 + c < ns) cm = fmaxf(cm, zm[c]);
        if (cm > mx) {
            const float r = expf(mx - cm);
            num *= r;
            den *= r;
            mx = cm;
        }
#pragma unroll
        for (int c = 0; c < 8; c++)
            if (z0 + c < ns) {
                const float f = expf(zm[c] - mx);
                den = fmaf(f, zl[c], den);
                num = fmaf(f, zv[c], num);
            }
    }
    const float v = den > 0.f ? num * (1.0f / den) : 0.f;
    if (!xs) {
        O[(size_t)q * ldo + h * HD + d] = v;
        return;
    }
    sv[d] = v;
    __syncthreads();
    if (d < HD / 8) {
        const float4 a = *reinterpret_cast<const float4*>(&sv[d * 8]), b = *reinterpret_cast<const float4*>(&sv[d * 8 + 4]);
        const float w[8] = {a.x, a.y, a.z, a.w, b.x, b.y, b.z, b.w};
        uint32_t hp[4], mp[4], lp[4];
#pragma unroll
        for (int e = 0; e < 8; e += 2) {
            uint16_t h0, m0, l0, h1, m1, l1;
            split3(w[e], h0, m0, l0);
            split3(w[e + 1], h1, m1, l1);
            hp[e / 2] = h0 | ((uint32_t)h1 << 16);
            mp[e / 2] = m0 | ((uint32_t)m1 << 16);
            lp[e / 2] = l0 | ((uint32_t)l1 << 16);
        }
        const int K = gridDim.x * HD, k = h * HD + d * 8;
        *reinterpret_cast<uint4*>(xs + frag_at(q, K, 0, k)) = make_uint4(hp[0], hp[1], hp[2], hp[3]);
        *reinterpret_cast<uint4*>(xs + frag_at(q, K, 1, k)) = make_uint4(mp[0], mp[1], mp[2], mp[3]);
        *reinterpret_cast<uint4*>(xs + frag_at(q, K, 2, k)) = make_uint4(lp[0], lp[1], lp[2], lp[3]);
    }
}

__device__ __forceinline__ void alt_row(float v, int r, float& am, float& as, float (&tv)[4], int (&ti)[4]) {
    if (v > am) {
        as = as * expf(am - v) + 1.0f;
        am = v;
    } else {
        as += expf(v - am);
    }
    if (r >= ALT_TEXT_MIN && v > tv[3]) {
        int k = 3;
        while (k > 0 && v > tv[k - 1]) {
            tv[k] = tv[k - 1];
            ti[k] = ti[k - 1];
            k--;
        }
        tv[k] = v;
        ti[k] = r;
    }
}

template <int EPI, int RB>
__device__ __forceinline__ void gemv_rows(int g, int (&rows)[RB]) {
#pragma unroll
    for (int i = 0; i < RB; i++) {
        if (EPI == EPI_SWIGLU) {
            const int u = g * (RB / 2) + (i >> 1);
            rows[i] = ((u >> 4) << 5) + (u & 15) + ((i & 1) << 4);
        } else {
            rows[i] = g * RB + i;
        }
    }
}

typedef unsigned int u32x4 __attribute__((ext_vector_type(4)));
template <int RB, int KQ>
__device__ __forceinline__ void gemv_load(__amdgpu_buffer_rsrc_t W, int rowbytes, const int (&rows)[RB],
                                          const int (&voff)[KQ], uint4 (&wv)[KQ][RB]) {
#pragma unroll
    for (int j = 0; j < KQ; j++)
#pragma unroll
        for (int i = 0; i < RB; i++) {
            const u32x4 v = __builtin_amdgcn_raw_buffer_load_b128(W, voff[j], rows[i] * rowbytes, 2);
            wv[j][i] = make_uint4(v.x, v.y, v.z, v.w);
        }
}

#ifdef VOX_GEMV_STAMPS
__device__ unsigned long long* g_gemv_stamps;
#define GEMV_STAMP(k) \
    do { if (g_gemv_stamps && tid == 0) g_gemv_stamps[(size_t)blockIdx.x * 4 + (k)] = __builtin_amdgcn_s_memrealtime(); } while (0)
#else
#define GEMV_STAMP(k) do {} while (0)
#endif

template <int PRO, int EPI, int RB, int KQ, int WQ8>
__global__ __launch_bounds__(256) void k_gemv(GemvArgs a) {
    constexpr int XPC = WQ8 ? 4 : 2;
    __shared__ float red[2][4][RB];
    __shared__ float sred[4];
    const int tid = threadIdx.x, lane = tid & 63, wave = tid >> 6;
    const int K = a.K, KC = WQ8 ? K >> 4 : K >> 3;
    const int ngroups = a.rows / RB;
    const int G = gridDim.x;
    int g = blockIdx.x;
    int rows[RB];
    uint4 wv[KQ][RB];
    float wsc[RB];
    GEMV_STAMP(0);
    bool first_group = true;
    const int rowbytes = K * (WQ8 ? 1 : 2);
    const __amdgpu_buffer_rsrc_t wrs =
        __builtin_amdgcn_make_buffer_rsrc(const_cast<void*>(a.W), 0, a.rows * rowbytes, 0x00020000);
    const __amdgpu_buffer_rsrc_t wnone = __builtin_amdgcn_make_buffer_rsrc(const_cast<void*>(a.W), 0, 0, 0x00020000);
    int voff[KQ];
#pragma unroll
    for (int j = 0; j < KQ; j++) {
        const int c0 = (j * 4 + wave) * 64 + lane;
        voff[j] = (c0 < KC ? c0 : 0) * 16;
    }
    gemv_rows<EPI, RB>(g, rows);
    gemv_load<RB, KQ>(wrs, rowbytes, rows, voff, wv);
    if ((EPI == EPI_LOGITS || EPI == EPI_LOGITS_ALT) && WQ8 && wave == 0) {
#pragma unroll
        for (int i = 0; i < RB; i++) wsc[i] = a.wscale[rows[i]];
    }

    float4 xr[KQ][XPC];
    constexpr bool EARLY = PRO != PRO_NONE && !WQ8;
    constexpr int NXP = EARLY ? XPC : 1;
    float4 nwr[KQ][NXP], adr[KQ][NXP];
    float ss = 0.f;
#pragma unroll
    for (int j = 0; j < KQ; j++) {
        const int c = (j * 4 + wave) * 64 + lane;
        const float4* xp = reinterpret_cast<const float4*>(a.x) + XPC * (c < KC ? c : 0);
        const float4 z = make_float4(0.f, 0.f, 0.f, 0.f);
#pragma unroll
        for (int h = 0; h < XPC; h++) {
            const float4 xv = xp[h];
            xr[j][h] = c < KC ? xv : z;
        }
        if (EARLY) {
            const int cc = c < KC ? c : 0;
            const float4* wp = reinterpret_cast<const float4*>(a.norm_w) + XPC * cc;
            const float4* ap = reinterpret_cast<const float4*>(PRO == PRO_NORM_ADA ? a.ada : a.norm_w) + XPC * cc;
#pragma unroll
            for (int h = 0; h < NXP; h++) {
                nwr[j][h] = wp[h];
                if (PRO == PRO_NORM_ADA) adr[j][h] = ap[h];
            }
        }
        if (PRO != PRO_NONE) {
#pragma unroll
            for (int h = 0; h < XPC; h++) {
                const float4 v = xr[j][h];
                ss = fmaf(v.x, v.x, fmaf(v.y, v.y, fmaf(v.z, v.z, fmaf(v.w, v.w, ss))));
            }
        }
    }
    if (PRO != PRO_NONE) {
        ss = wave_sum(ss);
        if (lane == 0) sred[wave] = ss;
        __syncthreads();
        const float tot = sred[0] + sred[1] + sred[2] + sred[3];
        const float inv = 1.0f / sqrtf(tot / (float)K + a.eps);
#pragma unroll
        for (int j = 0; j < KQ; j++) {
            const int c0 = (j * 4 + wave) * 64 + lane;
            const int c = c0 < KC ? c0 : 0;
            const float4* wp = reinterpret_cast<const float4*>(a.norm_w) + XPC * c;
            const float4* ap = reinterpret_cast<const float4*>(PRO == PRO_NORM_ADA ? a.ada : a.norm_w) + XPC * c;
#pragma unroll
            for (int h = 0; h < XPC; h++) {
                float4 v = xr[j][h];
                const float4 nw = EARLY ? nwr[j][h % NXP] : wp[h];
                v.x = v.x * inv * nw.x; v.y = v.y * inv * nw.y;
                v.z = v.z * inv * nw.z; v.w = v.w * inv * nw.w;
                if (PRO == PRO_NORM_ADA) {
                    const float4 ad = EARLY ? adr[j][h % NXP] : ap[h];
                    v.x *= (1.0f + ad.x); v.y *= (1.0f + ad.y);
                    v.z *= (1.0f + ad.z); v.w *= (1.0f + ad.w);
                }
                xr[j][h] = v;
            }
        }
    }

    constexpr bool QKVE = (EPI == EPI_QKV || EPI == EPI_QKV_BIAS);
    int lp = 0;
    if (QKVE) lp = a.state ? a.state[0] : a.pos;
    float best = -INFINITY;
    int besti = 0x7fffffff;
    float am = -INFINITY, as = 0.f, tv[4] = {-INFINITY, -INFINITY, -INFINITY, -INFINITY};
    int ti[4] = {-1, -1, -1, -1};
    constexpr bool LOGIT = (EPI == EPI_LOGITS || EPI == EPI_LOGITS_ALT);
    constexpr bool PAIRED = (QKVE || EPI == EPI_SWIGLU);
    constexpr int NL = LOGIT ? 1 : (PAIRED ? RB / 2 : RB);
    const bool owner = wave == 0 && lane < NL;
    const int i0 = PAIRED ? 2 * lane : lane;
    int buf = 0;
    for (;;) {
        const int gcur = g;
        int er0 = 0, er1 = 0;
        float ein0 = 0.f, ein1 = 0.f, esc0 = 1.f, esc1 = 1.f, eb0 = 0.f, eb1 = 0.f;
        if (!LOGIT && owner) {
            int rr[RB];
            gemv_rows<EPI, RB>(gcur, rr);
#pragma unroll
            for (int i = 0; i < RB; i++) {
                if (i == i0) er0 = rr[i];
                if (i == i0 + 1) er1 = rr[i];
            }
            if (WQ8) {
                esc0 = a.wscale[er0];
                if (PAIRED) esc1 = a.wscale[er1];
            }
            if (EPI == EPI_RESID) ein0 = a.y[er0] + (a.bias ? a.bias[er0] : 0.f);
            if (EPI == EPI_STORE) ein0 = a.bias ? a.bias[er0] : 0.f;
            if (EPI == EPI_QKV_BIAS) {
                eb0 = a.bias[er0];
                eb1 = a.bias[er1];
            }
            if (QKVE && er0 < a.qd + a.kvd) {
                const int col = er0 < a.qd ? er0 : er0 - a.qd;
                const float* rp = a.rope + (size_t)lp * a.hd + ((col % a.hd) & ~1);
                ein0 = rp[0];
                ein1 = rp[1];
            }
        }
        float acc[RB];
#pragma unroll
        for (int i = 0; i < RB; i++) acc[i] = 0.f;
#pragma unroll
        for (int j = 0; j < KQ; j++)
#pragma unroll
            for (int i = 0; i < RB; i++) {
                if (WQ8) acc[i] = dot16q(wv[j][i], reinterpret_cast<const float4(&)[4]>(xr[j]), acc[i]);
                else acc[i] = dot8(wv[j][i], xr[j][0], xr[j][XPC - 1], acc[i]);
            }
        if (first_group) {
            GEMV_STAMP(1);
            first_group = false;
        }
        int rcur[RB];
        float scur[RB];
        if (LOGIT) {
#pragma unroll
            for (int i = 0; i < RB; i++) {
                rcur[i] = rows[i];
                scur[i] = WQ8 ? wsc[i] : 1.0f;
            }
        }
        g += G;
        {
            const bool more = g < ngroups;
            gemv_rows<EPI, RB>(more ? g : 0, rows);
            gemv_load<RB, KQ>(more ? wrs : wnone, rowbytes, rows, voff, wv);
            if (LOGIT && WQ8 && wave == 0) {
#pragma unroll
                for (int i = 0; i < RB; i++) wsc[i] = a.wscale[rows[i]];
            }
        }
#pragma unroll
        for (int i = 0; i < RB; i++) acc[i] = wave_sum(acc[i]);
        if (lane == 0) {
#pragma unroll
            for (int i = 0; i < RB; i++) red[buf][wave][i] = acc[i];
        }
        __syncthreads();
        if (!LOGIT && owner) {
            float v0 = ((red[buf][0][i0] + red[buf][1][i0]) + red[buf][2][i0]) + red[buf][3][i0];
            float v1 = 0.f;
            if (PAIRED) v1 = ((red[buf][0][i0 + 1] + red[buf][1][i0 + 1]) + red[buf][2][i0 + 1]) + red[buf][3][i0 + 1];
            if (WQ8) {
                v0 *= esc0;
                v1 *= esc1;
            }
            if (EPI == EPI_QKV_BIAS) {
                v0 += eb0;
                v1 += eb1;
            }
            if (EPI == EPI_STORE || EPI == EPI_RESID) {
                a.y[er0] = ein0 + v0;
            } else if (EPI == EPI_SWIGLU) {
                a.y[gcur * (RB / 2) + lane] = silu(v0) * v1;
            } else if (QKVE) {
                if (er0 < a.qd + a.kvd) {
                    const float o0 = v0 * ein0 - v1 * ein1, o1 = v0 * ein1 + v1 * ein0;
                    if (er0 < a.qd) {
                        a.y[er0] = o0;
                        a.y[er1] = o1;
                    } else {
                        kv_st2_rt(a.Kc, (size_t)(lp % a.cap) * a.kvd + (er0 - a.qd), o0, o1, a.kv16);
                    }
                } else {
                    kv_st2_rt(a.Vc, (size_t)(lp % a.cap) * a.kvd + (er0 - a.qd - a.kvd), v0, v1, a.kv16);
                }
            }
        }
        if (LOGIT && wave == 0 && lane == 0) {
            float v[RB];
#pragma unroll
            for (int i = 0; i < RB; i++) {
                v[i] = ((red[buf][0][i] + red[buf][1][i]) + red[buf][2][i]) + red[buf][3][i];
                if (WQ8) v[i] *= scur[i];
            }
#pragma unroll
            for (int i = 0; i < RB; i++) {
                a.y[rcur[i]] = v[i];
                if (v[i] > best) { best = v[i]; besti = rcur[i]; }
                if (EPI == EPI_LOGITS_ALT) alt_row(v[i], rcur[i], am, as, tv, ti);
            }
        }
        buf ^= 1;
        if (g >= ngroups) break;
    }
    GEMV_STAMP(2);
    if ((EPI == EPI_LOGITS || EPI == EPI_LOGITS_ALT) && wave == 0 && lane == 0) {
        a.part_val[blockIdx.x] = best;
        a.part_idx[blockIdx.x] = besti;
        if (EPI == EPI_LOGITS_ALT) {
            float* pa = a.part_alt + (size_t)blockIdx.x * ALT_PART;
            pa[0] = am;
            pa[1] = as;
#pragma unroll
            for (int k = 0; k < 4; k++) {
                pa[2 + k] = tv[k];
                pa[6 + k] = __int_as_float(ti[k]);
            }
        }
    }
}

constexpr int ATT_CH = 16;
constexpr int ATT_WAVES = 16;
constexpr int ATT_BK = ATT_CH * ATT_WAVES;
constexpr int ATT_LWAVES = 8;
constexpr int ATT_LBK = ATT_CH * ATT_LWAVES;
constexpr int ATT_MIN_BK = 64;
constexpr int ATT_MAX_PARTS = 128;

template <int HD, int HPB, int DBG = 0, int FUSE = 0, int NWV = ATT_WAVES, class KT = float>
__global__ __launch_bounds__(NWV * 64) void k_attn_decode(const AttnPtrs P, int cap, int pos_host,
                                                          int window, float scale, int H, int KVH,
                                                          int maxs, const AttnFuse F = AttnFuse{}, int kvfast = 0) {
    constexpr int NT = NWV * 64, BK = NWV * ATT_CH;
    const int zb = blockIdx.z;
    const BatchSlot* __restrict__ sl = P.slots ? P.slots + zb : nullptr;
    if (sl && !sl->live) return;
    const float* __restrict__ q = P.q[zb];
    const KT* __restrict__ Kc = reinterpret_cast<const KT*>(sl ? sl->Kc + P.ring_off : (const char*)P.Kc[zb]);
    const KT* __restrict__ Vc = reinterpret_cast<const KT*>(sl ? sl->Vc + P.ring_off : (const char*)P.Vc[zb]);
    const int* __restrict__ state = sl ? nullptr : P.state[zb];
    float* __restrict__ part = P.part[zb];
    float* __restrict__ out = P.out[zb];
    constexpr int DQ = HD / 4;
    constexpr int DPL = HD / 64;
    __shared__ __attribute__((aligned(16))) float sQ[HPB][HD];
    __shared__ float sM[NWV][4], sL[NWV][4];
    __shared__ __attribute__((aligned(16))) float sO[NWV][HPB][HD];
    __shared__ __attribute__((aligned(16))) float sKn[FUSE ? HD : 1], sVn[FUSE ? HD : 1];
    const int hpk = H / KVH;
    const int kvh = HPB == 1 ? (int)blockIdx.y % KVH : kvfast ? (int)blockIdx.x % KVH : (int)blockIdx.y;
    const int h0 = HPB == 1 ? kvh * hpk + (int)blockIdx.y / KVH : kvh * hpk;
    const int nh = HPB == 1 ? 1 : hpk;
    const int sb = (HPB != 1 && kvfast) ? (int)blockIdx.x / KVH : (int)blockIdx.x;
    const int tid = threadIdx.x, lane = tid & 63, wave = tid >> 6;
    const int kvd = KVH * HD;
    unsigned long long ts[10];
    if (DBG == 4) {
        ts[0] = __builtin_amdgcn_s_memtime();
        ts[8] = __builtin_amdgcn_s_memrealtime();
    }
    auto dbg_dump = [&]() {
        if (DBG == 4) {
            ts[5] = __builtin_amdgcn_s_memtime();
            ts[9] = __builtin_amdgcn_s_memrealtime();
            if (lane == 0) {
                const size_t bi = P.slots ? (((size_t)blockIdx.z * gridDim.y + blockIdx.y) * gridDim.x + blockIdx.x) * NWV
                                          : (size_t)blockIdx.y * 16;
                unsigned long long* d = reinterpret_cast<unsigned long long*>(FUSE ? P.out[0] : P.part[0]) + (bi + wave) * 10;
                for (int i = 0; i < 10; i++) d[i] = ts[i];
            }
        }
    };
    constexpr int QPT = (HPB * HD + NT - 1) / NT;
    float qreg[QPT];
#pragma unroll
    for (int i = 0; i < QPT; i++) qreg[i] = (!FUSE && tid + i * NT < nh * HD) ? q[(size_t)h0 * HD + tid + i * NT] : 0.f;
    const int lp = sl ? sl->pos : state ? state[0] : pos_host;
    const int L = min(lp + 1, window);
    const int first = lp - L + 1;
    const int S = (L + BK - 1) / BK;
    if (sb >= S) return;
    const int k0 = first + sb * BK + wave * ATT_CH;
    const int kn = min(ATT_CH, lp + 1 - k0);
    const int kk = lane & 15, dq = lane >> 4;
    const int slot0 = k0 % cap;

    constexpr bool KROW = (HD == 128);
    float4 kv[DQ / 4];
    float vv[ATT_CH][DPL];
    {
        if (KROW) {
#pragma unroll
            for (int i = 0; i < DQ / 4; i++) {
                const int key = (lane >> 3) + 8 * (i & 1);
                int sk = slot0 + (key < kn ? key : 0);
                sk = sk >= cap ? sk - cap : sk;
                kv[i] = kv_ld4(Kc + (size_t)sk * kvd + kvh * HD + (i >> 1) * DQ + (lane & 7) * 4);
// ... 1724 lines not shown
    dim3 grid(N / G2_N, (M + G2_M - 1) / G2_M, 1);
    return wscale ? gemm2_launch<EPI, 1>(grid, st, A, lda, W, K, M, N, wscale, bias, C, ldc)
                  : gemm2_launch<EPI, 0>(grid, st, A, lda, W, K, M, N, wscale, bias, C, ldc);
}

hipError_t launch_gemm(int epi, int nsplit, const float* A, int lda, const void* W,
                       const float* wscale, int K, int M, int N, const float* bias, float* C,
                       int ldc, hipStream_t st, float* ws, size_t ws_elems) {
    if (M <= 0) return hipSuccess;
    if (nsplit != 3 || N % G2_N || K % G2_K || lda % 4) return hipErrorInvalidValue;
#define GEMM_CASE(E) \
    if (epi == E) return gemm_t<E>(A, lda, W, wscale, K, M, N, bias, C, ldc, st, ws, ws_elems);
    GEMM_CASE(EPI_STORE) GEMM_CASE(EPI_RESID) GEMM_CASE(EPI_GELU) GEMM_CASE(EPI_GELU_ERF) GEMM_CASE(EPI_SWIGLU)
#undef GEMM_CASE
    return hipErrorInvalidValue;
}

hipError_t launch_rope_kv(const float* qkv, int M, int qd, int kvd, int hd, const float* rope,
                          int pos0, float* q, float* Kc, float* Vc, int cap, hipStream_t st, int kv16) {
    if (M <= 0) return hipSuccess;
    if (kvd % 2) return hipErrorInvalidValue;
    if (kv16)
        hipLaunchKernelGGL(k_rope_kv<kvh_t>, dim3(M), dim3(256), 0, st, qkv, M, qd, kvd, hd, rope, pos0, q, Kc, Vc, cap);
    else
        hipLaunchKernelGGL(k_rope_kv<float>, dim3(M), dim3(256), 0, st, qkv, M, qd, kvd, hd, rope, pos0, q, Kc, Vc, cap);
    LAUNCH_CHECK();
    return hipSuccess;
}

VOX_KB_KNOB(g_attn_blocks, 0);

hipError_t launch_rope_kv_rows(const float* qkv, int N, int qd, int kvd, int hd, const float* rope_table,
                               const EncRows& er, float* q, int cap, hipStream_t st) {
    if (N <= 0) return hipSuccess;
    if (er.B < 1 || er.B > VOX_MAX_BATCH) return hipErrorInvalidValue;
    hipLaunchKernelGGL(k_rope_kv_rows, dim3(N), dim3(256), 0, st, qkv, qd, kvd, hd, rope_table, er, q, cap);
    LAUNCH_CHECK();
    return hipSuccess;
}

static int g_att_planes = -1;
static bool att_planes() {
    if (g_att_planes < 0) {
        const char* e = getenv("VOX_HIP_ATT_PLANES");
        g_att_planes = (e && atoi(e) == 0) ? 0 : 1;
    }
    return g_att_planes == 1;
}

hipError_t launch_attn_rows(int hd, const float* Q, const EncRows& er, int N, int cap, float* O, int H, int KVH,
                            int window, float scale, float* ws, size_t ws_elems, hipStream_t st, uint16_t* xs) {
    if (N <= 0) return hipSuccess;
    if (er.B < 1 || er.B > VOX_MAX_BATCH || (hd != 64 && hd != 128)) return hipErrorInvalidValue;
    if (xs && N > PLANE_MAX_ROWS) return hipErrorInvalidValue;
    int qbm = 0, keys = 0;
    for (int b = 0; b < er.B; b++) {
        qbm = std::max(qbm, (er.nr[b] + 15) / 16);
        const int ks = std::max(er.pos0[b] - window + 1, 0);
        keys = std::max(keys, er.pos0[b] + er.nr[b] - ks);
    }
    if (qbm == 0) return hipSuccess;
    int ns = 1;
    int nblk = 0;
    for (int b = 0; b < er.B; b++) nblk += H * ((er.nr[b] + 15) / 16);
    if (ws && nblk < 256) {
        ns = std::min((keys + 63) / 64, std::max(1, 256 / nblk));
        while (ns > 1 && (size_t)H * N * ns * (hd + 2) > ws_elems) ns--;
    }
    dim3 grid(H, qbm, ns * er.B);
    uint16_t* kxs = ns == 1 && att_planes() ? xs : nullptr;
    if (hd == 64)
        hipLaunchKernelGGL((k_attn_mf<64, float, 1>), grid, dim3(256), 0, st, Q, H * hd, nullptr, nullptr, cap, O, H * hd,
                           N, H, KVH, 0, 0, window, scale, ns, ws, er, kxs);
    else
        hipLaunchKernelGGL((k_attn_mf<128, float, 1>), grid, dim3(256), 0, st, Q, H * hd, nullptr, nullptr, cap, O,
                           H * hd, N, H, KVH, 0, 0, window, scale, ns, ws, er, kxs);
    LAUNCH_CHECK();
    if (ns > 1) {
        if (hd == 64)
            hipLaunchKernelGGL(k_attn_tiled_combine<64>, dim3(H, N), dim3(64), 0, st, ws, ns, N, O, H * hd, xs);
        else
            hipLaunchKernelGGL(k_attn_tiled_combine<128>, dim3(H, N), dim3(128), 0, st, ws, ns, N, O, H * hd, xs);
        LAUNCH_CHECK();
    } else if (xs && !kxs) {
        return launch_split_fplanes(O, N, H * hd, xs, st);
    }
    return hipSuccess;
}

hipError_t launch_attn_rows_mf(int hd, const float* Q, int ldq, const float* Kc, const float* Vc,
                             int cap, float* O, int ldo, int M, int H, int KVH, int q_pos0,
                             int k_first, int window, float scale, hipStream_t st, float* ws, size_t ws_elems,
                             uint16_t* xs, int kv16) {
    if (M <= 0) return hipSuccess;
    if (hd != 64 && hd != 128) return hipErrorInvalidValue;
    if (xs && (M > PLANE_MAX_ROWS || ldo != H * hd)) return hipErrorInvalidValue;
    const int QT = 16;
    const int qb = (M + QT - 1) / QT;
    int ks = q_pos0 - window + 1;
    if (ks < k_first) ks = k_first;
    const int keys = q_pos0 + M - ks;
    int ns = 1;
    if (ws && H * qb < 256) {
        const int target = g_attn_blocks ? g_attn_blocks : 256;
        ns = std::min((keys + 63) / 64, std::max(1, target / (H * qb)));
        while (ns > 1 && (size_t)H * M * ns * (hd + 2) > ws_elems) ns--;
    }
    dim3 grid(H, qb, ns);
    if (kv16) {
        if (hd != 128) return hipErrorInvalidValue;
        hipLaunchKernelGGL((k_attn_mf<128, kvh_t>), grid, dim3(256), 0, st, Q, ldq, Kc, Vc, cap, O, ldo, M, H, KVH,
                           q_pos0, k_first, window, scale, ns, ws);
    } else if (hd == 64) {
        hipLaunchKernelGGL(k_attn_mf<64>, grid, dim3(256), 0, st, Q, ldq, Kc, Vc, cap, O, ldo, M, H, KVH, q_pos0,
                           k_first, window, scale, ns, ws, EncRows{}, ns == 1 && att_planes() ? xs : nullptr);
    } else {
        hipLaunchKernelGGL(k_attn_mf<128>, grid, dim3(256), 0, st, Q, ldq, Kc, Vc, cap, O, ldo, M, H, KVH, q_pos0,
                           k_first, window, scale, ns, ws, EncRows{}, ns == 1 && att_planes() ? xs : nullptr);
    }
    LAUNCH_CHECK();
    if (ns > 1) {
        if (hd == 64)
            hipLaunchKernelGGL(k_attn_tiled_combine<64>, dim3(H, M), dim3(64), 0, st, ws, ns, M, O, ldo, xs);
        else
            hipLaunchKernelGGL(k_attn_tiled_combine<128>, dim3(H, M), dim3(128), 0, st, ws, ns, M, O, ldo, xs);
        LAUNCH_CHECK();
    } else if (xs && (kv16 || !att_planes())) {
        return launch_split_fplanes(O, M, H * hd, xs, st);
    }
    return hipSuccess;
}

hipError_t launch_slabs_rope_kv(const float* part, int S, int M, const float* bias, int qd, int kvd, int hd,
                                const float* rope, int pos0, float* q, float* Kc, float* Vc, int cap, hipStream_t st) {
    if (M <= 0) return hipSuccess;
    if (M > SK_MAX_ROWS || S < 1 || qd % hd || kvd % hd || hd % 2) return hipErrorInvalidValue;
    hipLaunchKernelGGL(k_slabs_rope_kv, dim3((qd / 2 + kvd + 255) / 256, M), dim3(256), 0, st, part, S, bias, qd, kvd,
                       hd, rope, pos0, q, Kc, Vc, cap);
    LAUNCH_CHECK();
    return hipSuccess;
}

#ifdef VOX_GEMV_STAMPS
hipError_t gemv_set_stamps(unsigned long long* p) { return hipMemcpyToSymbol(HIP_SYMBOL(g_gemv_stamps), &p, sizeof p); }
#endif
VOX_KB_KNOB(g_gemv_rb, 0);
static int gemv_rb(int rows) {
    if (g_gemv_rb && rows % g_gemv_rb == 0) return g_gemv_rb;
    if (rows >= 65536 && rows % 8 == 0) return 8;
    if (rows >= 6144 && rows % 4 == 0) return 4;
    return 2;
}

VOX_KB_KNOB(g_gemv_maxb, 0);
int gemv_grid(int rows) {
    const int ng = rows / gemv_rb(rows), maxb = g_gemv_maxb ? g_gemv_maxb : GEMV_MAX_BLOCKS;
    int best = 1;
    for (int gsz = 1; gsz <= maxb && gsz <= ng; gsz++)
        if (ng % gsz == 0) best = gsz;
    if (best < 256 && ng > maxb) best = maxb;
    return best;
}

template <int P, int E, int RB, int Q8>
static const void* gemv_fn(int kq) {
    switch (kq) {
        case 1: return reinterpret_cast<const void*>(&k_gemv<P, E, RB, 1, Q8>);
        case 2: return reinterpret_cast<const void*>(&k_gemv<P, E, RB, 2, Q8>);
        case 3: return reinterpret_cast<const void*>(&k_gemv<P, E, RB, 3, Q8>);
        case 4: return reinterpret_cast<const void*>(&k_gemv<P, E, RB, 4, Q8>);
        case 5: return reinterpret_cast<const void*>(&k_gemv<P, E, RB, 5, Q8>);
        default: return nullptr;
    }
}

int gemv_occupancy(const void* fn) {
    int occ = 0;
    if (hipOccupancyMaxActiveBlocksPerMultiprocessor(&occ, fn, 256, 0) != hipSuccess) occ = 0;
    return occ;
}

template <int P, int E, int RB, int Q8>
static hipError_t gemv_k(const GemvArgs& a, int grid, hipStream_t st) {
    const int kq = ((Q8 ? a.K >> 4 : a.K >> 3) + 255) / 256;
    switch (kq) {
#define KQ_CASE(Q) case Q: hipLaunchKernelGGL((k_gemv<P, E, RB, Q, Q8>), dim3(grid), dim3(256), 0, st, a); break;
        KQ_CASE(1) KQ_CASE(2) KQ_CASE(3) KQ_CASE(4) KQ_CASE(5)
#undef KQ_CASE
        default: return hipErrorInvalidValue;
    }
    LAUNCH_CHECK();
    return hipSuccess;
}

const void* gemv_kernel(int pro, int epi, const GemvArgs& a) {
    const int rb = gemv_rb(a.rows);
    const int kq = ((a.wscale ? a.K >> 4 : a.K >> 3) + 255) / 256;
#define GEMV_FN(P, E)                                                                     \
    if (pro == P && epi == E)                                                             \
        return rb == 8 ? (a.wscale ? gemv_fn<P, E, 8, 1>(kq) : gemv_fn<P, E, 8, 0>(kq))   \
             : rb == 2 ? (a.wscale ? gemv_fn<P, E, 2, 1>(kq) : gemv_fn<P, E, 2, 0>(kq))   \
                       : (a.wscale ? gemv_fn<P, E, 4, 1>(kq) : gemv_fn<P, E, 4, 0>(kq));
    GEMV_FN(PRO_NONE, EPI_STORE) GEMV_FN(PRO_NONE, EPI_RESID) GEMV_FN(PRO_NORM, EPI_QKV)
    GEMV_FN(PRO_NORM_ADA, EPI_SWIGLU) GEMV_FN(PRO_NORM, EPI_LOGITS) GEMV_FN(PRO_NORM, EPI_LOGITS_ALT)
    GEMV_FN(PRO_NORM, EPI_QKV_BIAS) GEMV_FN(PRO_NORM, EPI_SWIGLU)
#undef GEMV_FN
    return nullptr;
}

template <int P, int E, int RB>
static hipError_t gemv_q(const GemvArgs& a, int grid, hipStream_t st) {
    return a.wscale ? gemv_k<P, E, RB, 1>(a, grid, st) : gemv_k<P, E, RB, 0>(a, grid, st);
}

hipError_t launch_gemv_timed(int pro, int epi, const GemvArgs& a, hipEvent_t start, hipEvent_t stop,
                             hipStream_t st) {
    const void* fn = gemv_kernel(pro, epi, a);
    if (!fn) return hipErrorInvalidValue;
    GemvArgs args = a;
    void* kargs[] = {&args};
    return hipExtLaunchKernel(fn, dim3(gemv_grid(a.rows)), dim3(256), kargs, 0, st, start, stop, 0);
}

bool gemv_ok(int rows, int K, int q8) {
    const int kc = q8 ? K >> 4 : K >> 3;
    return rows > 0 && K > 0 && K % (q8 ? 16 : 8) == 0 && rows % gemv_rb(rows) == 0 && (kc + 255) / 256 <= 5;
}

hipError_t launch_gemv(int pro, int epi, const GemvArgs& a, hipStream_t st) {
    const int rb = gemv_rb(a.rows);
    if (!gemv_ok(a.rows, a.K, a.wscale != nullptr)) return hipErrorInvalidValue;
    if (epi == EPI_QKV_BIAS && !a.bias) return hipErrorInvalidValue;
    const int grid = gemv_grid(a.rows);
#define GEMV_CASE(P, E) \
    if (pro == P && epi == E)                                                            \
        return rb == 8 ? gemv_q<P, E, 8>(a, grid, st) : rb == 2 ? gemv_q<P, E, 2>(a, grid, st) : gemv_q<P, E, 4>(a, grid, st);
    GEMV_CASE(PRO_NONE, EPI_STORE) GEMV_CASE(PRO_NONE, EPI_RESID) GEMV_CASE(PRO_NORM, EPI_QKV)
    GEMV_CASE(PRO_NORM_ADA, EPI_SWIGLU) GEMV_CASE(PRO_NORM, EPI_LOGITS) GEMV_CASE(PRO_NORM, EPI_LOGITS_ALT)
    GEMV_CASE(PRO_NORM, EPI_QKV_BIAS) GEMV_CASE(PRO_NORM, EPI_SWIGLU)
#undef GEMV_CASE
    return hipErrorInvalidValue;
}

int attn_maxch(int window) { return std::max(4, (window + ATT_MIN_BK - 1) / ATT_MIN_BK); }
int attn_maxsplits(int window) { return (window + ATT_BK - 1) / ATT_BK; }
VOX_KB_KNOB(g_attn_lw, 0);
VOX_KB_KNOB(g_attn_kvfast, 1);
int g_attn_bsplit = -1;

template <int HD, int NWV, class KT>
static void attn_long(const AttnPtrs& p, int nb, int cap, int pos_host, int window, float scale, int H, int KVH,
                      int splits, int maxs, hipStream_t st) {
    const int nsb = splits * (ATT_BK / (NWV * ATT_CH));
    if (g_attn_kvfast)
        hipLaunchKernelGGL((k_attn_decode<HD, 4, 0, 0, NWV, KT>), dim3(nsb * KVH, 1, nb), dim3(NWV * 64), 0, st, p,
                           cap, pos_host, window, scale, H, KVH, maxs, AttnFuse{}, 1);
    else
        hipLaunchKernelGGL((k_attn_decode<HD, 4, 0, 0, NWV, KT>), dim3(nsb, KVH, nb), dim3(NWV * 64), 0, st, p, cap,
                           pos_host, window, scale, H, KVH, maxs);
}

template <class KT>
static hipError_t attn_launch(int hd, const AttnPtrs& p, int nb, int cap, int pos_host, int window, float scale,
                              int H, int KVH, int splits, hipStream_t st) {
    const int maxs = attn_maxch(window);
    if (H % KVH || H / KVH > 4 || maxs > ATT_MAX_PARTS || splits < 1 || splits > attn_maxsplits(window) || nb < 1 ||
        nb > VOX_MAX_BATCH)
        return hipErrorInvalidValue;
#define VOX_ATT(HD)                                                                                        \
    if (splits == 1 && nb >= 4) {                                                                         \
        hipLaunchKernelGGL((k_attn_decode<HD, 4, 0, 0, ATT_WAVES, KT>), dim3(1, KVH, nb), dim3(1024), 0, st, p, \
                           cap, pos_host, window, scale, H, KVH, maxs);                                    \
    } else if (splits == 1) {                                                                              \
        hipLaunchKernelGGL((k_attn_decode<HD, 1, 0, 0, ATT_WAVES, KT>), dim3(1, H, nb), dim3(1024), 0, st, p,   \
                           cap, pos_host, window, scale, H, KVH, maxs);                                    \
    } else if (g_attn_lw == 4 || (g_attn_lw == 2 && splits * 8 <= maxs)) {                                \
        if (g_attn_lw == 4) attn_long<HD, 4, KT>(p, nb, cap, pos_host, window, scale, H, KVH, splits, maxs, st); \
        else attn_long<HD, 2, KT>(p, nb, cap, pos_host, window, scale, H, KVH, splits, maxs, st);          \
    } else if (g_attn_lw == 16) {                                                                          \
        attn_long<HD, 16, KT>(p, nb, cap, pos_host, window, scale, H, KVH, splits, maxs, st);              \
    } else {                                                                                               \
        attn_long<HD, ATT_LWAVES, KT>(p, nb, cap, pos_host, window, scale, H, KVH, splits, maxs, st);      \
    }
    if (hd == 128) {
        VOX_ATT(128)
    } else if (hd == 64 && sizeof(KT) == 4) {
        VOX_ATT(64)
    } else {
        return hipErrorInvalidValue;
    }
#undef VOX_ATT
    LAUNCH_CHECK();
    return hipSuccess;
}

int g_attn_short = -1;
hipError_t launch_attn_decode(int hd, const float* q, const float* Kc, const float* Vc, int cap,
                              const int* state, int pos_host, int window, float scale, int H,
                              int KVH, float* part, float* out, int splits, hipStream_t st, int kv16) {
    if (g_attn_short < 0) {
        const char* e = getenv("VOX_HIP_ATT_SHORT");
        g_attn_short = (e && atoi(e) == 0) ? 0 : 1;
    }
    if (g_attn_short && splits == 1 && hd == 128 && window > ATT_BK && cap >= ATT_BK && H % KVH == 0) {
        if (kv16)
            hipLaunchKernelGGL((k_attn_short<128, kvh_t, 4>), dim3(H), dim3(1024), 0, st, q,
                               reinterpret_cast<const kvh_t*>(Kc), reinterpret_cast<const kvh_t*>(Vc), state, pos_host,
                               scale, H, KVH, out);
        else
            hipLaunchKernelGGL((k_attn_short<128, float, 4>), dim3(H), dim3(1024), 0, st, q, Kc, Vc, state, pos_host,
                               scale, H, KVH, out);
        LAUNCH_CHECK();
        return hipSuccess;
    }
    AttnPtrs p;
    memset(&p, 0, sizeof p);
    p.q[0] = q; p.Kc[0] = Kc; p.Vc[0] = Vc; p.state[0] = state; p.part[0] = part; p.out[0] = out;
    return kv16 ? attn_launch<kvh_t>(hd, p, 1, cap, pos_host, window, scale, H, KVH, splits, st)
                : attn_launch<float>(hd, p, 1, cap, pos_host, window, scale, H, KVH, splits, st);
}

hipError_t launch_attn_decode_batch(int hd, const AttnPtrs& p, int nb, int cap, int window, float scale,
                                    int H, int KVH, int splits, hipStream_t st, int kv16) {
    return kv16 ? attn_launch<kvh_t>(hd, p, nb, cap, 0, window, scale, H, KVH, splits, st)
                : attn_launch<float>(hd, p, nb, cap, 0, window, scale, H, KVH, splits, st);
}

template <class KT>
static hipError_t attn_batch_fused(const AttnPtrs& p, const AttnFuse& f, int nb, int cap, int window, float scale,
                                   int H, int KVH, int splits, int maxs, hipStream_t st) {
    if (g_attn_bsplit < 0) {
        const char* e = getenv("VOX_HIP_ATT_BSPLIT");
        g_attn_bsplit = e ? std::max(0, std::min(2, atoi(e))) : 1;
    }
    if (splits == 1 && (!g_attn_bsplit || (g_attn_bsplit == 1 && nb * KVH >= 256))) {
        hipLaunchKernelGGL((k_attn_decode<128, 4, 0, 1, ATT_WAVES, KT>), dim3(1, KVH, nb), dim3(1024), 0, st, p, cap, 0,
                           window, scale, H, KVH, maxs, f);
        LAUNCH_CHECK();
        return hipSuccess;
    }
    hipLaunchKernelGGL((k_attn_decode<128, 4, 0, 1, ATT_LWAVES, KT>), dim3(splits * (ATT_BK / ATT_LBK) * KVH, 1, nb),
                       dim3(ATT_LWAVES * 64), 0, st, p, cap, 0, window, scale, H, KVH, maxs, f, 1);
    LAUNCH_CHECK();
    return hipSuccess;
}

hipError_t launch_attn_batch_fused(int hd, const AttnPtrs& p, const AttnFuse& f, int nb, int cap, int window,
                                   float scale, int H, int KVH, int splits, hipStream_t st, int kv16) {
    const int maxs = attn_maxch(window);
    if (hd != 128 || H % KVH || H / KVH > 4 || maxs > ATT_MAX_PARTS || splits < 1 || splits > attn_maxsplits(window) ||
        nb < 1 || nb > VOX_MAX_BATCH || !f.qkv || !f.rope || !f.xs || f.S < 1 || f.N != (H + 2 * KVH) * hd)
        return hipErrorInvalidValue;
    return kv16 ? attn_batch_fused<kvh_t>(p, f, nb, cap, window, scale, H, KVH, splits, maxs, st)
                : attn_batch_fused<float>(p, f, nb, cap, window, scale, H, KVH, splits, maxs, st);
}
hipError_t launch_attn_batch_dbg(const AttnPtrs& p, const AttnFuse& f, int nb, int cap, int window, float scale, int H,
                                 int KVH, int splits, hipStream_t st) {
    const int maxs = attn_maxch(window);
    if (!p.out[0] || nb < 1 || nb > VOX_MAX_BATCH || H % KVH || H / KVH > 4) return hipErrorInvalidValue;
    hipLaunchKernelGGL((k_attn_decode<128, 4, 4, 1, ATT_LWAVES, float>), dim3(splits * (ATT_BK / ATT_LBK) * KVH, 1, nb),
                       dim3(ATT_LWAVES * 64), 0, st, p, cap, 0, window, scale, H, KVH, maxs, f, 1);
    LAUNCH_CHECK();
    return hipSuccess;
}
hipError_t launch_attn_dbg(int dbg, const float* q, const float* Kc, const float* Vc, int cap,
// ... 360 lines not shown
```

voxtral.c_amd/csrc/vox_synth.c:

```c
#include <math.h>
#include <stddef.h>
#include <stdint.h>
#include <string.h>

static inline uint64_t splitmix64(uint64_t x) {
    x += 0x9E3779B97F4A7C15ull;
    x = (x ^ (x >> 30)) * 0xBF58476D1CE4E5B9ull;
    x = (x ^ (x >> 27)) * 0x94D049BB133111EBull;
    return x ^ (x >> 31);
}

static inline float unif(uint64_t seed, uint64_t i) {
    uint64_t h = splitmix64(seed ^ splitmix64(i));
    return (float)((h >> 40) * (1.0 / 16777216.0)) * 2.0f - 1.0f;
}

void vox_synth_bf16(uint16_t *out, size_t n, uint64_t seed, float std, float offset) {
    const float a = std * 1.7320508075688772f;
#pragma omp parallel for schedule(static)
    for (long long i = 0; i < (long long)n; i++) {
        float v = offset + a * unif(seed, (uint64_t)i);
        uint32_t u;
        memcpy(&u, &v, 4);
        u += 0x7fffu + ((u >> 16) & 1u);
        out[i] = (uint16_t)(u >> 16);
    }
}

void vox_synth_f32(float *out, size_t n, uint64_t seed, float lo, float hi) {
#pragma omp parallel for schedule(static)
    for (long long i = 0; i < (long long)n; i++) {
        float u = 0.5f * (unif(seed, (uint64_t)i) + 1.0f);
        out[i] = lo + (hi - lo) * u;
    }
}

void vox_bf16_to_f32(float *out, const uint16_t *in, size_t n) {
#pragma omp parallel for schedule(static)
    for (long long i = 0; i < (long long)n; i++) {
        uint32_t u = ((uint32_t)in[i]) << 16;
        memcpy(&out[i], &u, 4);
    }
}

void vox_quantize_q8_bf16(const uint16_t *in, long long rows, long long cols, float *scales,
                          int8_t *q) {
#pragma omp parallel for schedule(dynamic, 16)
    for (long long r = 0; r < rows; r++) {
        const uint16_t *src = in + r * cols;
        int8_t *dst = q + r * cols;
        float amax = 0.0f;
        for (long long c = 0; c < cols; c++) {
            uint32_t u = ((uint32_t)src[c]) << 16;
            float v;
            memcpy(&v, &u, 4);
            v = fabsf(v);
            if (v > amax) amax = v;
        }
        if (amax == 0.0f) {
            scales[r] = 0.0f;
            memset(dst, 0, (size_t)cols);
            continue;
        }
        const float s = (float)((double)amax / 127.0);
        scales[r] = s;
        for (long long c = 0; c < cols; c++) {
            uint32_t u = ((uint32_t)src[c]) << 16;
            float v;
            memcpy(&v, &u, 4);
            float t = rintf(v / s);
            t = t < -128.0f ? -128.0f : (t > 127.0f ? 127.0f : t);
            dst[c] = (int8_t)t;
        }
    }
}

void vox_dequant_q8(float *out, const int8_t *q, const float *scales, long long rows, long long cols) {
#pragma omp parallel for schedule(static)
    for (long long r = 0; r < rows; r++)
        for (long long c = 0; c < cols; c++) out[r * cols + c] = (float)q[r * cols + c] * scales[r];
}
```

voxtral.c_amd/vox_hip.py:

```python
from __future__ import annotations

import ctypes
import os

import numpy as np

from vox_weights import (VoxConfig, Weights, build_weights_struct, config_struct_class,
                         weights_struct_class)

_HERE = os.path.dirname(os.path.abspath(__file__))
LIB_PATH = os.environ.get("VOX_HIP_LIB") or os.path.join(_HERE, "libvoxtral_hip.so")

TOKEN_BOS, TOKEN_EOS, TOKEN_STREAMING_PAD = 1, 2, 32
STREAM_FIRST_CHUNK_MIN_MEL = 312
STREAM_DEFAULT_INTERVAL = 2.0
RAW_AUDIO_LENGTH_PER_TOK = 1280
OFFLINE_STREAMING_BUFFER_TOKENS = 10

ConfigC = config_struct_class()
WeightsC = weights_struct_class()

EXPORTS = [
    "vox_hip_init", "vox_hip_available", "vox_hip_shutdown", "vox_hip_memory_used",
    "vox_hip_last_error", "vox_hip_clear_error", "vox_hip_set_device", "vox_hip_config_voxtral_4b",
    "vox_hip_model_create", "vox_hip_model_free", "vox_hip_model_set_delay",
    "vox_hip_model_ada_scale", "vox_hip_model_set_kv_fp16", "vox_hip_stream_kv_fp16",
    "vox_hip_set_gemm_planes", "vox_hip_gemm_planes", "vox_hip_set_gemmf_wait",
    "vox_hip_stream_create", "vox_hip_stream_free",
    "vox_hip_stream_reset", "vox_hip_stream_reset_decoder", "vox_hip_stream_encode_mel",
    "vox_hip_stream_adapter_tokens", "vox_hip_stream_read_adapter", "vox_hip_stream_decode",
    "vox_hip_batch_create", "vox_hip_batch_free", "vox_hip_batch_decode", "vox_hip_batch_decode_rows",
    "vox_hip_batch_begin_rows", "vox_hip_batch_finish",
    "vox_hip_batch_read_logits",
    "vox_hip_batch_stats",
    "vox_hip_stream_state", "vox_hip_stream_set_alt", "vox_hip_stream_read_alts", "vox_hip_sgemm_bf16", "vox_hip_sgemm_q8", "vox_hip_fused_qkv_bf16",
    "vox_hip_fused_ffn_bf16", "vox_hip_encoder_attention", "vox_hip_encoder_full_step",
    "vox_hip_decoder_prefill_step", "vox_hip_decoder_start", "vox_hip_decoder_end",
    "vox_hip_decoder_full_step", "vox_hip_stream_set_profiling", "vox_hip_stream_profile",
    "vox_hip_stream_sync", "vox_hip_stream_set_async_encode", "vox_hip_stream_encode_mel_batch", "vox_hip_device_upload", "vox_hip_device_free",
    "vox_hip_mel_create", "vox_hip_mel_feed", "vox_hip_mel_finish", "vox_hip_mel_frames",
    "vox_hip_mel_frame_ptr", "vox_hip_mel_discard_before", "vox_hip_mel_read", "vox_hip_mel_free", "vox_hip_mel_reset",
]

_lib = None


def lib():
    global _lib
    if _lib is not None:
        return _lib
    if not os.path.exists(LIB_PATH):
        raise RuntimeError(f"{LIB_PATH} not built (run __graft_entry__.build())")
    L = ctypes.CDLL(LIB_PATH)
    P, I, F = ctypes.c_void_p, ctypes.c_int, ctypes.c_float
    fp = ctypes.POINTER(ctypes.c_float)
    ip = ctypes.POINTER(ctypes.c_int)
    sig = {
        "vox_hip_init": (I, []), "vox_hip_available": (I, []), "vox_hip_shutdown": (None, []),
        "vox_hip_memory_used": (ctypes.c_size_t, []), "vox_hip_last_error": (ctypes.c_char_p, []),
        "vox_hip_clear_error": (None, []),
        "vox_hip_set_device": (I, [I]),
        "vox_hip_config_voxtral_4b": (None, [P]),
        "vox_hip_model_create": (P, [P, P, I]), "vox_hip_model_free": (None, [P]),
        "vox_hip_model_set_delay": (I, [P, I]), "vox_hip_model_ada_scale": (I, [P, fp]),
        "vox_hip_model_set_kv_fp16": (I, [P, I]), "vox_hip_stream_kv_fp16": (I, [P]),
        "vox_hip_set_gemm_planes": (I, [I]), "vox_hip_gemm_planes": (I, []),
        "vox_hip_set_gemmf_wait": (I, [I]),
        "vox_hip_stream_create": (P, [P]), "vox_hip_stream_free": (None, [P]),
        "vox_hip_stream_reset": (I, [P]), "vox_hip_stream_reset_decoder": (I, [P]),
        "vox_hip_stream_encode_mel": (I, [P, P, I, I]),
        "vox_hip_stream_adapter_tokens": (I, [P]),
        "vox_hip_stream_read_adapter": (I, [P, I, I, fp]),
        "vox_hip_stream_decode": (I, [P, I, I, ip, fp]),
        "vox_hip_stream_state": (I, [P, ip]),
        "vox_hip_batch_create": (P, [P, I]), "vox_hip_batch_free": (None, [P]),
        "vox_hip_batch_decode": (I, [P, ctypes.POINTER(ctypes.c_void_p), I, I, I, ip, ip]),
        "vox_hip_batch_decode_rows": (I, [P, ctypes.POINTER(ctypes.c_void_p), I, ip, I, I, ip, ip]),
        "vox_hip_batch_begin_rows": (I, [P, ctypes.POINTER(ctypes.c_void_p), I, ip, I, I, ip, ip]),
        "vox_hip_batch_finish": (I, [P]),
        "vox_hip_batch_read_logits": (I, [P, P, fp]),
        "vox_hip_batch_stats": (I, [P, ctypes.POINTER(ctypes.c_longlong)]),
        "vox_hip_stream_set_alt": (I, [P, I, F]),
        "vox_hip_stream_read_alts": (I, [P, I, I, ip, fp]),
        "vox_hip_sgemm_bf16": (None, [I, I, I, fp, P, fp]),
        "vox_hip_sgemm_q8": (None, [I, I, I, fp, P, fp, fp]),
        "vox_hip_fused_qkv_bf16": (None, [I, I, fp, P, I, P, I, P, I, fp, fp, fp]),
        "vox_hip_fused_ffn_bf16": (None, [I, I, I, fp, P, P, P, fp]),
        "vox_hip_encoder_attention": (None, [fp, fp, fp, fp, I, I, I, I, I, F, I, I]),
        "vox_hip_encoder_full_step": (I, [P, fp, I, fp, I]),
        "vox_hip_decoder_prefill_step": (I, [P, fp, I, fp, I]),
        "vox_hip_decoder_start": (None, [P, fp, I]), "vox_hip_decoder_end": (None, [P]),
        "vox_hip_decoder_full_step": (I, [P, fp, I, fp]),
        "vox_hip_stream_set_profiling": (I, [P, I]),
        "vox_hip_stream_profile": (I, [P, ctypes.POINTER(ctypes.c_double)]),
        "vox_hip_stream_sync": (I, [P]),
        "vox_hip_stream_set_async_encode": (I, [P, I]),
        "vox_hip_stream_encode_mel_batch": (I, [P, P, P, I, I, P]),
        "vox_hip_device_upload": (P, [P, ctypes.c_size_t]),
        "vox_hip_device_free": (I, [P]),
        "vox_hip_mel_create": (P, [P, I]), "vox_hip_mel_feed": (I, [P, fp, I]),
        "vox_hip_mel_finish": (I, [P, I]), "vox_hip_mel_frames": (I, [P, ip]),
        "vox_hip_mel_frame_ptr": (P, [P, I]), "vox_hip_mel_discard_before": (I, [P, I]),
        "vox_hip_mel_read": (I, [P, I, I, fp]), "vox_hip_mel_free": (None, [P]), "vox_hip_mel_reset": (I, [P, I]),
    }
    for name, (res, args) in sig.items():
        fn = getattr(L, name)
        fn.restype = res
        fn.argtypes = args
    _lib = L
    return L


def fptr(a: np.ndarray):
    assert a.dtype == np.float32 and a.flags.c_contiguous
    return a.ctypes.data_as(ctypes.POINTER(ctypes.c_float))


def _err(what):
    msg = lib().vox_hip_last_error()
    raise RuntimeError(f"{what}: {msg.decode() if msg else 'unknown error'}")


def set_gemm_planes(planes: int):
    if lib().vox_hip_set_gemm_planes(int(planes)) != 0:
        _err("set_gemm_planes")


def gemm_planes() -> int:
    return lib().vox_hip_gemm_planes()


def set_gemmf_wait(ticks: int) -> int:
    return lib().vox_hip_set_gemmf_wait(int(ticks))


def init(device: int | None = None):
    L = lib()
    if device is not None and L.vox_hip_set_device(device) != 0:
        _err("set_device")
    if not L.vox_hip_init():
        _err("vox_hip_init (no GPU?)")


class Model:

    def __init__(self, cfg: VoxConfig, weights: Weights, delay_tokens: int = 6):
        init()
        self.cfg = cfg
        self.delay_tokens = delay_tokens
        self._cfg_c = cfg.ctypes_struct(ConfigC)
        wstruct, keep = build_weights_struct(weights, WeightsC)
        self.h = lib().vox_hip_model_create(ctypes.byref(self._cfg_c), ctypes.byref(wstruct), delay_tokens)
        if not self.h:
            _err("vox_hip_model_create")

    def set_delay(self, delay_ms: int):
        delay_ms = min(max(delay_ms, 80), 2400)
        self.delay_tokens = delay_ms // 80
        if lib().vox_hip_model_set_delay(self.h, self.delay_tokens) != 0:
            _err("set_delay")

    def set_kv_fp16(self, on: bool):
        if lib().vox_hip_model_set_kv_fp16(self.h, int(on)) != 0:
            _err("set_kv_fp16")

    def ada_scale(self):
        c = self.cfg
        out = np.empty(c.dec_layers * c.dec_dim, np.float32)
        lib().vox_hip_model_ada_scale(self.h, fptr(out))
        return out.reshape(c.dec_layers, c.dec_dim)

    def close(self):
        if self.h:
            lib().vox_hip_model_free(self.h)
            self.h = None


def encode_mel_batch(streams, mels):
    n = len(streams)
    assert n == len(mels) and n > 0
    arrs = [np.ascontiguousarray(m, dtype=np.float32) for m in mels]
    for s, a in zip(streams, arrs):
        assert a.ndim == 2 and a.shape[1] == s.cfg.mel_bins, (a.shape, s.cfg.mel_bins)
        assert s.model is streams[0].model, "encode_mel_batch: streams of one model"
    hs = (ctypes.c_void_p * n)(*[s.h for s in streams])
    ps = (ctypes.c_void_p * n)(*[a.ctypes.data for a in arrs])
    ns = np.array([a.shape[0] for a in arrs], np.int32)
    added = np.zeros(n, np.int32)
    if lib().vox_hip_stream_encode_mel_batch(hs, ps, ns.ctypes.data, n, 0, added.ctypes.data) != 0:
        _err("encode_mel_batch")
    return added.tolist()


class Stream:

    def __init__(self, model: Model):
        self.model = model
        self.cfg = model.cfg
        self.h = lib().vox_hip_stream_create(model.h)
        if not self.h:
            _err("vox_hip_stream_create")

    def reset(self):
        if lib().vox_hip_stream_reset(self.h) != 0:
            _err("reset")

    @property
    def kv_fp16(self) -> bool:
        return bool(lib().vox_hip_stream_kv_fp16(self.h))

    def encode_mel(self, mel: np.ndarray) -> int:
        mel = np.ascontiguousarray(mel, dtype=np.float32)
        assert mel.ndim == 2 and mel.shape[1] == self.cfg.mel_bins
        n = lib().vox_hip_stream_encode_mel(self.h, mel.ctypes.data, mel.shape[0], 0)
        if n < 0:
            _err("encode_mel")
        return n

    def encode_mel_device(self, dev_ptr: int, n_frames: int) -> int:
        n = lib().vox_hip_stream_encode_mel(self.h, ctypes.c_void_p(dev_ptr), n_frames, 1)
        if n < 0:
            _err("encode_mel")
        return n

    def set_async_encode(self, on: bool):
        if lib().vox_hip_stream_set_async_encode(self.h, int(on)) != 0:
            _err("set_async_encode")

    def sync(self):
        if lib().vox_hip_stream_sync(self.h) != 0:
            _err("sync")

    @property
    def adapter_tokens(self) -> int:
        return lib().vox_hip_stream_adapter_tokens(self.h)

    def read_adapter(self, first: int = 0, n: int | None = None) -> np.ndarray:
        if n is None:
            n = self.adapter_tokens - first
        out = np.empty((n, self.cfg.dec_dim), np.float32)
        if n and lib().vox_hip_stream_read_adapter(self.h, first, n, fptr(out)) != 0:
            _err("read_adapter")
        return out

    def decode(self, max_steps: int = 1 << 30, stop_at_eos: bool = True, want_logits: bool = False):
        max_steps = min(max_steps, 1 << 20)
        cap = min(max_steps, max(self.adapter_tokens + 1, 1))
        toks = np.zeros(cap, np.int32)
        logits = np.zeros((cap, self.cfg.vocab), np.float32) if want_logits else None
        n = lib().vox_hip_stream_decode(self.h, cap, int(stop_at_eos),
                                        toks.ctypes.data_as(ctypes.POINTER(ctypes.c_int)),
                                        fptr(logits) if want_logits else None)
        if n < 0:
            _err("decode")
        return (toks[:n], logits[:n]) if want_logits else toks[:n]

    def state(self):
        o = np.zeros(6, np.int32)
        lib().vox_hip_stream_state(self.h, o.ctypes.data_as(ctypes.POINTER(ctypes.c_int)))
        return dict(zip(["kv_pos", "gen_pos", "prev_token", "started", "eos_seen", "generated"], o.tolist()))

    def set_alt(self, n_alt: int, cutoff: float):
        if lib().vox_hip_stream_set_alt(self.h, n_alt, cutoff) != 0:
            _err("set_alt")

    def read_alts(self, first: int, n: int):
        ids = np.empty((n, 4), np.int32)
        pr = np.empty((n, 4), np.float32)
        if lib().vox_hip_stream_read_alts(self.h, first, n, ids.ctypes.data_as(ctypes.POINTER(ctypes.c_int)),
                                          fptr(pr)) != 0:
            _err("read_alts")
        return ids, pr

    def twin_encoder_full_step(self, x: np.ndarray, rope: np.ndarray, logical_start: int) -> np.ndarray:
        x = np.array(x, np.float32, copy=True, order="C")
        rope = np.ascontiguousarray(rope, np.float32)
        if lib().vox_hip_encoder_full_step(self.h, fptr(x), x.shape[0], fptr(rope), logical_start) != 0:
            _err("encoder_full_step")
        return x

    def twin_decoder_prefill_step(self, x: np.ndarray, rope: np.ndarray, logical_start: int) -> np.ndarray:
        x = np.array(x, np.float32, copy=True, order="C")
        rope = np.ascontiguousarray(rope, np.float32)
        if lib().vox_hip_decoder_prefill_step(self.h, fptr(x), x.shape[0], fptr(rope), logical_start) != 0:
            _err("decoder_prefill_step")
        return x

    def twin_decoder_step(self, x: np.ndarray, rope_row: np.ndarray, logical_pos: int, want_logits=True):
        x = np.ascontiguousarray(x, np.float32)
        rope_row = np.ascontiguousarray(rope_row, np.float32)
        L = lib()
        L.vox_hip_clear_error()
        L.vox_hip_decoder_start(self.h, fptr(x), x.shape[-1])
        if L.vox_hip_last_error():
            _err("decoder_start")
        logits = np.empty(self.cfg.vocab, np.float32) if want_logits else None
        tok = L.vox_hip_decoder_full_step(self.h, fptr(rope_row), logical_pos,
                                          fptr(logits) if want_logits else None)
        L.vox_hip_decoder_end(self.h)
        if tok < 0:
            _err("decoder_full_step")
        return tok, logits

    def set_profiling(self, on: bool):
        lib().vox_hip_stream_set_profiling(self.h, int(on))

    def profile(self):
        o = (ctypes.c_double * 8)()
        lib().vox_hip_stream_profile(self.h, o)
        return {"ms": o[0], "bytes": o[1], "launches": int(o[2]), "avg_ms": o[3], "kind": int(o[4]),
                "bytes_per_launch": o[5], "gemmf_recomputes": int(o[6])}

    def sync(self):
        lib().vox_hip_stream_sync(self.h)

    def close(self):
        if self.h:
            lib().vox_hip_stream_free(self.h)
# ... 403 lines not shown
```

Baseline: 681.5.

## Pack decoder bf16 weights into lossless 13-bit format for GEMV decode

At load time, each decoder weight matrix and the LM head is scanned for its exponent range. When the exponents fit a 5-bit window, the bf16 values are repacked losslessly into 13-bit codes: a 12-byte main record per 8 weights plus a side stream of high bits laid out per row group. The GEMV kernel gains a packed-weight variant that loads 96-bit records plus side words and rebuilds fp16 values in registers before the FMAs. This cuts weight bytes read per decode token by about 19%, which targets a memory-bound decoder, at the cost of extra ALU bit manipulation, longer model load, and a new layout that must stay consistent with the kernel.

```diff
diff --git a/include/voxtral_hip.h b/include/voxtral_hip.h
--- a/include/voxtral_hip.h
+++ b/include/voxtral_hip.h
@@ -50,6 +50,16 @@
 int vox_hip_model_set_delay(vox_hip_model_t *m, int delay_tokens);
 int vox_hip_model_ada_scale(vox_hip_model_t *m, float *out);
 int vox_hip_model_set_kv_fp16(vox_hip_model_t *m, int on);
+typedef struct {
+    int packed_tensors;
+    int raw_tensors;
+    long long packed_bytes;
+    long long packed_raw_bytes;
+    long long raw_bytes;
+    double pack_ms;
+} vox_hip_wpack_stats_t;
+int vox_hip_model_wpack_stats(const vox_hip_model_t *m, vox_hip_wpack_stats_t *out);
+int vox_hip_gemv_wpack(int rows, int K, const uint16_t *W, const float *x, float *y, int packed);
 int vox_hip_set_gemm_planes(int planes);
 int vox_hip_gemm_planes(void);
 int vox_hip_set_gemmf_wait(int ticks);
diff --git a/voxtral.c_amd/csrc/vox_hip.hip b/voxtral.c_amd/csrc/vox_hip.hip
--- a/voxtral.c_amd/csrc/vox_hip.hip
+++ b/voxtral.c_amd/csrc/vox_hip.hip
@@ -1,5 +1,6 @@
 #include "../../include/voxtral_hip.h"
 #include "vox_hip_internal.h"
+#include "vox_wpack.h"
 
 #include <hip/hip_runtime.h>
 #include <math.h>
@@ -11,8 +12,10 @@
 #include <stddef.h>
 #include <algorithm>
 #include <atomic>
+#include <chrono>
 #include <mutex>
 #include <string>
+#include <thread>
 #include <unordered_map>
 #include <vector>
 
@@ -120,10 +123,15 @@
     float *sqkv, *so, *s13, *s2;
     float *bqkv, *bo, *b2, *attn_norm, *ffn_norm;
 };
+struct WPackD {
+    uint8_t *main, *side;
+    int d;
+};
 struct DecLayerD {
     uint8_t *wqkv, *wo, *w13, *w2;
     float *sqkv, *so, *s13, *s2;
     float *attn_norm, *ffn_norm;
+    WPackD pqkv, po, p13, p2;
 };
 struct DecFragD {
     uint8_t *wqkv, *wo, *w13, *w2;
@@ -151,6 +159,9 @@
     std::vector<DecFragD> efrag;
     uint8_t* lm_frag;
     int kv16;
+    WPackD plm;
+    int wpack;
+    vox_hip_wpack_stats_t wstats;
 };
 
 static int upload(void* dst, const void* src, size_t bytes) {
@@ -221,6 +232,55 @@
     return 0;
 }
 
+template <class F>
+static void par_range(long long n, F f) {
+    const long long nt = std::max(1LL, std::min<long long>({16, (long long)std::thread::hardware_concurrency(), n}));
+    std::vector<std::thread> th;
+    for (long long t = 1; t < nt; t++) th.emplace_back([=] { f(n * t / nt, n * (t + 1) / nt); });
+    f(0, n / nt);
+    for (auto& t : th) t.join();
+}
+
+static int wpack_make(int enabled, vox_hip_wpack_stats_t& S, WPackD* P, const uint16_t* w, int rows, int K, int swiglu) {
+    P->main = P->side = nullptr;
+    P->d = 0;
+    const size_t n = (size_t)rows * K;
+    auto raw = [&] { S.raw_tensors++; S.raw_bytes += (long long)n * 2; return 0; };
+    if (!w) return set_err("null weight pointer");
+    if (!enabled || !gemv_ok(rows, K, 0)) return raw();
+    const auto t0 = std::chrono::steady_clock::now();
+    int lo = 256, hi = -1, bad = 0;
+    std::mutex mu;
+    par_range(rows, [&](long long r0, long long r1) {
+        int l = 256, h = -1, b = 0;
+        vox_wpack13_scan_range(w + r0 * K, (size_t)(r1 - r0) * K, &l, &h, &b);
+        std::lock_guard<std::mutex> g(mu);
+        lo = std::min(lo, l); hi = std::max(hi, h); bad |= b;
+    });
+    int d;
+    if (!vox_wpack13_choose(lo, hi, bad, &d)) return raw();
+    const int rb = gemv_rowgroup(rows), sw = vox_wpack13_side_words(K, rb);
+    const size_t mainw = n / 8 * 3, sidew = (size_t)rows / rb * 256 * sw;
+    std::vector<uint32_t> hm(mainw), hs(sidew);
+    std::vector<uint8_t> hb(n / 8);
+    par_range(rows, [&](long long r0, long long r1) { vox_wpack13_pack_rows(w, r0, r1, K, d, hm.data(), hb.data()); });
+    par_range(rows / rb, [&](long long g0, long long g1) { vox_wpack13_side_groups(hb.data(), g0, g1, K, rb, swiglu, hs.data()); });
+    CK(dalloc(&P->main, mainw * 4));
+    CK(dalloc(&P->side, sidew * 4));
+    if (upload(P->main, hm.data(), mainw * 4) || upload(P->side, hs.data(), sidew * 4)) return -1;
+    P->d = d;
+    S.packed_tensors++;
+    S.packed_bytes += (long long)(mainw + sidew) * 4;
+    S.packed_raw_bytes += (long long)n * 2;
+    S.pack_ms += std::chrono::duration<double, std::milli>(std::chrono::steady_clock::now() - t0).count();
+    return 0;
+}
+static void wpack_args(GemvArgs& a, const WPackD& P) {
+    a.wp_main = P.main;
+    a.wp_side = P.side;
+    a.wp_d = P.d;
+}
+
 static int model_update_ada(vox_hip_model_t* m) {
     const vox_hip_config_t& c = m->c;
     int D = c.dec_dim, A = c.ada_dim;
@@ -306,6 +366,12 @@
     m->ad0_s = m->ad1_s = m->tok_emb_s = nullptr;
     m->conv0_b = m->conv1_b = m->enc_norm = m->dec_norm = m->ada_scale = nullptr;
     m->rope_enc = m->rope_dec = nullptr;
+    memset(&m->plm, 0, sizeof m->plm);
+    memset(&m->wstats, 0, sizeof m->wstats);
+    {
+        const char* e = getenv("VOX_HIP_WPACK");
+        m->wpack = (e && atoi(e) == 0) ? 0 : 1;
+    }
     const vox_hip_config_t& c = *cfg;
     const int ED = c.enc_dim, EQ = c.enc_heads * c.enc_head_dim, EKV = c.enc_kv_heads * c.enc_head_dim;
     const int EH = c.enc_hidden;
@@ -349,6 +415,8 @@
     TRY(upload_mat(&m->ad0, &m->ad0_s, w->ad0, w->ad0_s, DD, (size_t)ED * c.downsample));
     TRY(upload_mat(&m->ad1, &m->ad1_s, w->ad1, w->ad1_s, DD, DD));
     TRY(upload_mat(&m->tok_emb, &m->tok_emb_s, w->tok_emb, w->tok_emb_s, c.vocab, DD));
+    if (!w->tok_emb_s) TRY(wpack_make(m->wpack, m->wstats, &m->plm, (const uint16_t*)w->tok_emb, c.vocab, DD, 0));
+    std::vector<uint16_t> hrows;
     m->dec.resize(c.dec_layers);
     m->ada_down.resize(c.dec_layers);
     m->ada_up.resize(c.dec_layers);
@@ -360,6 +428,24 @@
         TRY(upload_mat(&L.wo, &L.so, w->dec_wo[l], SCL(dec_wo_s, l), DD, DQ));
         TRY(upload_w13(&L.w13, &L.s13, w->dec_w1[l], SCL(dec_w1_s, l), w->dec_w3[l], SCL(dec_w3_s, l), DH, DD));
         TRY(upload_mat(&L.w2, &L.s2, w->dec_w2[l], SCL(dec_w2_s, l), DD, DH));
+        if (!L.sqkv) {
+            hrows.resize((size_t)(DQ + 2 * DKV) * DD);
+            memcpy(hrows.data(), w->dec_wq[l], (size_t)DQ * DD * 2);
+            memcpy(hrows.data() + (size_t)DQ * DD, w->dec_wk[l], (size_t)DKV * DD * 2);
+            memcpy(hrows.data() + (size_t)(DQ + DKV) * DD, w->dec_wv[l], (size_t)DKV * DD * 2);
+            TRY(wpack_make(m->wpack, m->wstats, &L.pqkv, hrows.data(), DQ + 2 * DKV, DD, 0));
+        }
+        if (!L.so) TRY(wpack_make(m->wpack, m->wstats, &L.po, (const uint16_t*)w->dec_wo[l], DD, DQ, 0));
+        if (!L.s13) {
+            hrows.resize((size_t)2 * DH * DD);
+            const size_t grp = (size_t)16 * DD;
+            for (int g = 0; g < DH / 16; g++) {
+                memcpy(hrows.data() + 2 * g * grp, (const uint16_t*)w->dec_w1[l] + g * grp, grp * 2);
+                memcpy(hrows.data() + (2 * g + 1) * grp, (const uint16_t*)w->dec_w3[l] + g * grp, grp * 2);
+            }
+            TRY(wpack_make(m->wpack, m->wstats, &L.p13, hrows.data(), 2 * DH, DD, 1));
+        }
+        if (!L.s2) TRY(wpack_make(m->wpack, m->wstats, &L.p2, (const uint16_t*)w->dec_w2[l], DD, DH, 0));
         TRYH(dalloc(&L.attn_norm, DD));
         TRY(upload(L.attn_norm, w->dec_attn_norm[l], DD * 4));
         TRYH(dalloc(&L.ffn_norm, DD));
@@ -391,7 +477,9 @@
         dfree(L.wqkv); dfree(L.wo); dfree(L.w13); dfree(L.w2);
         dfree(L.sqkv); dfree(L.so); dfree(L.s13); dfree(L.s2);
         dfree(L.attn_norm); dfree(L.ffn_norm);
-    }
+        for (WPackD* P : {&L.pqkv, &L.po, &L.p13, &L.p2}) { dfree(P->main); dfree(P->side); }
+    }
+    dfree(m->plm.main); dfree(m->plm.side);
     for (auto& F : m->dfrag) {
         dfree(F.wqkv); dfree(F.wo); dfree(F.w13); dfree(F.w2);
     }
@@ -403,6 +491,12 @@
     dfree(m->ad0_s); dfree(m->ad1_s); dfree(m->tok_emb_s);
     dfree(m->ada_scale); dfree(m->rope_enc); dfree(m->rope_dec);
     delete m;
+}
+
+extern "C" int vox_hip_model_wpack_stats(const vox_hip_model_t* m, vox_hip_wpack_stats_t* out) {
+    if (!m || !out) return set_err("wpack_stats: null argument");
+    *out = m->wstats;
+    return 0;
 }
 
 extern "C" int vox_hip_model_set_delay(vox_hip_model_t* m, int delay_tokens) {
@@ -1726,20 +1820,24 @@
         a.state = state; a.pos = pos;
         a.rope = state ? m->rope_dec : rope_row - (size_t)pos * hd;
         a.Kc = Kc; a.Vc = Vc; a.cap = s->dcap; a.kv16 = s->kv16;
+        wpack_args(a, L.pqkv);
         CK(launch_gemv(PRO_NORM, EPI_QKV, a, st));
         CK(launch_attn_decode(hd, s->qd_, Kc, Vc, s->dcap, state, pos, c.dec_window, scale, H, KVH,
                               s->part, s->attd, splits, st, s->kv16));
         memset(&a, 0, sizeof a);
         a.x = s->attd; a.K = DQ; a.W = L.wo; a.wscale = L.so; a.rows = DD; a.y = s->xd;
+        wpack_args(a, L.po);
         CK(launch_gemv(PRO_NONE, EPI_RESID, a, st));
         memset(&a, 0, sizeof a);
         a.x = s->xd; a.K = DD; a.W = L.w13; a.wscale = L.s13; a.rows = 2 * DH; a.norm_w = L.ffn_norm;
         a.ada = m->ada_scale + (size_t)l * DD; a.eps = c.dec_eps; a.y = s->gated;
+        wpack_args(a, L.p13);
         const bool gprof = s->profiling && state && !s->capturing && (int)s->pev.size() == 2 * c.dec_layers;
         if (gprof) CK(launch_gemv_timed(PRO_NORM_ADA, EPI_SWIGLU, a, s->pev[2 * l], s->pev[2 * l + 1], st));
         else CK(launch_gemv(PRO_NORM_ADA, EPI_SWIGLU, a, st));
         memset(&a, 0, sizeof a);
         a.x = s->gated; a.K = DH; a.W = L.w2; a.wscale = L.s2; a.rows = DD; a.y = s->xd;
+        wpack_args(a, L.p2);
         CK(launch_gemv(PRO_NONE, EPI_RESID, a, st));
     }
     return enqueue_lm_head(s, state);
@@ -1754,6 +1852,7 @@
     a.x = s->xd; a.K = c.dec_dim; a.W = m->tok_emb; a.wscale = m->tok_emb_s; a.rows = c.vocab; a.norm_w = m->dec_norm;
     a.eps = c.dec_eps; a.y = s->logits; a.part_val = s->pval; a.part_idx = s->pidx;
     a.part_alt = s->part_alt;
+    wpack_args(a, m->plm);
     CK(launch_gemv(PRO_NORM, (state && s->n_alt > 1) ? EPI_LOGITS_ALT : EPI_LOGITS, a, st));
     return 0;
 }
@@ -2129,6 +2228,37 @@
         return -1;
     CK(hipStreamSynchronize(g_twin_st));
     return 0;
+}
+
+extern "C" int vox_hip_gemv_wpack(int rows, int K, const uint16_t* W, const float* x, float* y, int packed) {
+    std::lock_guard<std::mutex> lk(g_twin_mu);
+    if (!W || !x || !y) return set_err("gemv_wpack: null argument");
+    if (!gemv_ok(rows, K, 0)) return set_err("gemv_wpack: shape %d x %d is not a GEMV shape", rows, K);
+    if (twin_init()) return -1;
+    uint8_t* dW = nullptr;
+    float *dx = nullptr, *dy = nullptr;
+    WPackD P = {nullptr, nullptr, 0};
+    vox_hip_wpack_stats_t S;
+    memset(&S, 0, sizeof S);
+    auto run = [&]() -> int {
+        CK(dalloc(&dW, (size_t)rows * K * 2));
+        CK(dalloc(&dx, (size_t)K));
+        CK(dalloc(&dy, (size_t)rows));
+        if (upload(dW, W, (size_t)rows * K * 2) || upload(dx, x, (size_t)K * 4)) return -1;
+        if (wpack_make(packed, S, &P, W, rows, K, 0)) return -1;
+        GemvArgs a;
+        memset(&a, 0, sizeof a);
+        a.x = dx; a.K = K; a.W = dW; a.rows = rows; a.y = dy;
+        wpack_args(a, P);
+        CK(launch_gemv(PRO_NONE, EPI_STORE, a, g_twin_st));
+        CK(hipStreamSynchronize(g_twin_st));
+        CK(hipMemcpy(y, dy, (size_t)rows * 4, hipMemcpyDeviceToHost));
+        return 0;
+    };
+    const int rc = run();
+    const int was_packed = P.main != nullptr;
+    dfree(dW); dfree(dx); dfree(dy); dfree(P.main); dfree(P.side);
+    return rc ? -1 : was_packed;
 }
 
 extern "C" void vox_hip_sgemm_bf16(int M, int N, int K, const float* A, const uint16_t* B, float* C) {
diff --git a/voxtral.c_amd/csrc/vox_hip_dev.h b/voxtral.c_amd/csrc/vox_hip_dev.h
--- a/voxtral.c_amd/csrc/vox_hip_dev.h
+++ b/voxtral.c_amd/csrc/vox_hip_dev.h
@@ -140,6 +140,24 @@
     return acc;
 }
 
+__device__ __forceinline__ float hlo(uint32_t w) { return (float)__builtin_bit_cast(_Float16, (unsigned short)(w & 0xffffu)); }
+__device__ __forceinline__ float hhi(uint32_t w) { return (float)__builtin_bit_cast(_Float16, (unsigned short)(w >> 16)); }
+__device__ __forceinline__ float dot8h(uint4 w, uint32_t sd, int q, float4 a, float4 b, float acc) {
+    const uint32_t HM = 0xfff8fff8u, SM = 0x00070007u;
+    const uint32_t t = (w.x & SM) | ((w.y & SM) << 3) | ((w.z & SM) << 6);
+    const uint32_t p3 = (t << 3) | ((sd << (4 * q)) & 0xf000f000u);
+    const uint32_t p0 = w.x & HM, p1 = w.y & HM, p2 = w.z & HM;
+    acc = fmaf(hlo(p0), a.x, acc);
+    acc = fmaf(hhi(p0), a.y, acc);
+    acc = fmaf(hlo(p1), a.z, acc);
+    acc = fmaf(hhi(p1), a.w, acc);
+    acc = fmaf(hlo(p2), b.x, acc);
+    acc = fmaf(hhi(p2), b.y, acc);
+    acc = fmaf(hlo(p3), b.z, acc);
+    acc = fmaf(hhi(p3), b.w, acc);
+    return acc;
+}
+
 __device__ __forceinline__ float i8f(uint32_t w, int b) { return (float)((int32_t)(w << (24 - 8 * b)) >> 24); }
 __device__ __forceinline__ float dot16q(uint4 w, const float4 (&x)[4], float acc) {
     const uint32_t d[4] = {w.x, w.y, w.z, w.w};
diff --git a/voxtral.c_amd/csrc/vox_hip_internal.h b/voxtral.c_amd/csrc/vox_hip_internal.h
--- a/voxtral.c_amd/csrc/vox_hip_internal.h
+++ b/voxtral.c_amd/csrc/vox_hip_internal.h
@@ -12,6 +12,7 @@
 constexpr int ALT_PART = 10;
 constexpr int ALT_REC = 8;
 enum { PRO_NONE = 0, PRO_NORM = 1, PRO_NORM_ADA = 2 };
+enum { WF_BF16 = 0, WF_Q8 = 1, WF_P13 = 2 };
 
 constexpr int GEMV_MAX_BLOCKS = 1024;
 
@@ -20,6 +21,9 @@
     int K;
     const void* W;
     const float* wscale;
+    const void* wp_main = nullptr;
+    const void* wp_side = nullptr;
+    int wp_d = 0;
     int rows;
     const float* norm_w;
     const float* ada;
@@ -79,6 +83,7 @@
 constexpr int ARGB = 64;
 
 int gemv_grid(int rows);
+int gemv_rowgroup(int rows);
 bool gemv_ok(int rows, int K, int q8);
 int attn_maxch(int window);
 int attn_maxsplits(int window);
diff --git a/voxtral.c_amd/csrc/vox_hip_kernels.hip b/voxtral.c_amd/csrc/vox_hip_kernels.hip
--- a/voxtral.c_amd/csrc/vox_hip_kernels.hip
+++ b/voxtral.c_amd/csrc/vox_hip_kernels.hip
@@ -629,13 +629,19 @@
 }
 
 typedef unsigned int u32x4 __attribute__((ext_vector_type(4)));
-template <int RB, int KQ>
+typedef unsigned int u32x3 __attribute__((ext_vector_type(3)));
+template <int RB, int KQ, bool WP = false>
 __device__ __forceinline__ void gemv_load(__amdgpu_buffer_rsrc_t W, int rowbytes, const int (&rows)[RB],
                                           const int (&voff)[KQ], uint4 (&wv)[KQ][RB]) {
 #pragma unroll
     for (int j = 0; j < KQ; j++)
 #pragma unroll
         for (int i = 0; i < RB; i++) {
+            if constexpr (WP) {
+                const u32x3 v = __builtin_amdgcn_raw_buffer_load_b96(W, voff[j], rows[i] * rowbytes, 2);
+                wv[j][i] = make_uint4(v.x, v.y, v.z, 0u);
+                continue;
+            }
             const u32x4 v = __builtin_amdgcn_raw_buffer_load_b128(W, voff[j], rows[i] * rowbytes, 2);
             wv[j][i] = make_uint4(v.x, v.y, v.z, v.w);
         }
@@ -649,9 +655,36 @@
 #define GEMV_STAMP(k) do {} while (0)
 #endif
 
-template <int PRO, int EPI, int RB, int KQ, int WQ8>
+template <int SW>
+__device__ __forceinline__ void gemv_load_side(__amdgpu_buffer_rsrc_t S, int voff, int soff, uint32_t (&sd)[SW]) {
+    if constexpr (SW == 1) {
+        sd[0] = __builtin_amdgcn_raw_buffer_load_b32(S, voff, soff, 2);
+    } else if constexpr (SW == 2) {
+        const u32x2 v = __builtin_amdgcn_raw_buffer_load_b64(S, voff, soff, 2);
+        sd[0] = v.x; sd[1] = v.y;
+    } else if constexpr (SW == 3) {
+        const u32x3 v = __builtin_amdgcn_raw_buffer_load_b96(S, voff, soff, 2);
+        sd[0] = v.x; sd[1] = v.y; sd[2] = v.z;
+    } else {
+        static_assert(SW % 4 != 3, "side record size");
+#pragma unroll
+        for (int o = 0; o + 4 <= SW; o += 4) {
+            const u32x4 v = __builtin_amdgcn_raw_buffer_load_b128(S, voff + o * 4, soff, 2);
+            sd[o] = v.x; sd[o + 1] = v.y; sd[o + 2] = v.z; sd[o + 3] = v.w;
+        }
+        if constexpr (SW % 4 == 1) sd[SW - 1] = __builtin_amdgcn_raw_buffer_load_b32(S, voff + (SW - 1) * 4, soff, 2);
+        if constexpr (SW % 4 == 2) {
+            const u32x2 v = __builtin_amdgcn_raw_buffer_load_b64(S, voff + (SW - 2) * 4, soff, 2);
+            sd[SW - 2] = v.x; sd[SW - 1] = v.y;
+        }
+    }
+}
+
+template <int PRO, int EPI, int RB, int KQ, int WF>
 __global__ __launch_bounds__(256) void k_gemv(GemvArgs a) {
+    constexpr bool WQ8 = WF == WF_Q8, WP = WF == WF_P13;
     constexpr int XPC = WQ8 ? 4 : 2;
+    constexpr int SW = WP ? (KQ * RB + 3) / 4 : 1;
     __shared__ float red[2][4][RB];
     __shared__ float sred[4];
     const int tid = threadIdx.x, lane = tid & 63, wave = tid >> 6;
@@ -664,18 +697,23 @@
     float wsc[RB];
     GEMV_STAMP(0);
     bool first_group = true;
-    const int rowbytes = K * (WQ8 ? 1 : 2);
-    const __amdgpu_buffer_rsrc_t wrs =
-        __builtin_amdgcn_make_buffer_rsrc(const_cast<void*>(a.W), 0, a.rows * rowbytes, 0x00020000);
-    const __amdgpu_buffer_rsrc_t wnone = __builtin_amdgcn_make_buffer_rsrc(const_cast<void*>(a.W), 0, 0, 0x00020000);
+    const int rowbytes = WP ? KC * 12 : K * (WQ8 ? 1 : 2);
+    void* const wbase = const_cast<void*>(WP ? a.wp_main : a.W);
+    const __amdgpu_buffer_rsrc_t wrs = __builtin_amdgcn_make_buffer_rsrc(wbase, 0, a.rows * rowbytes, 0x00020000);
+    const __amdgpu_buffer_rsrc_t wnone = __builtin_amdgcn_make_buffer_rsrc(wbase, 0, 0, 0x00020000);
+    void* const sbase = const_cast<void*>(WP ? a.wp_side : a.W);
+    const __amdgpu_buffer_rsrc_t srs = __builtin_amdgcn_make_buffer_rsrc(sbase, 0, ngroups * (256 * SW * 4), 0x00020000);
+    const __amdgpu_buffer_rsrc_t snone = __builtin_amdgcn_make_buffer_rsrc(sbase, 0, 0, 0x00020000);
+    uint32_t sd[SW];
     int voff[KQ];
 #pragma unroll
     for (int j = 0; j < KQ; j++) {
         const int c0 = (j * 4 + wave) * 64 + lane;
-        voff[j] = (c0 < KC ? c0 : 0) * 16;
+        voff[j] = (c0 < KC ? c0 : 0) * (WP ? 12 : 16);
     }
     gemv_rows<EPI, RB>(g, rows);
-    gemv_load<RB, KQ>(wrs, rowbytes, rows, voff, wv);
+    if (WP) gemv_load_side<SW>(srs, tid * (SW * 4), g * (256 * SW * 4), sd);
+    gemv_load<RB, KQ, WP>(wrs, rowbytes, rows, voff, wv);
     if ((EPI == EPI_LOGITS || EPI == EPI_LOGITS_ALT) && WQ8 && wave == 0) {
 #pragma unroll
         for (int i = 0; i < RB; i++) wsc[i] = a.wscale[rows[i]];
@@ -740,6 +778,18 @@
                 xr[j][h] = v;
             }
         }
+    }
+
+    if (WP) {
+#pragma unroll
+        for (int j = 0; j < KQ; j++)
+#pragma unroll
+            for (int h = 0; h < XPC; h++) {
+                float4 v = xr[j][h];
+                v.x = ldexpf(v.x, a.wp_d); v.y = ldexpf(v.y, a.wp_d);
+                v.z = ldexpf(v.z, a.wp_d); v.w = ldexpf(v.w, a.wp_d);
+                xr[j][h] = v;
+            }
     }
 
     constexpr bool QKVE = (EPI == EPI_QKV || EPI == EPI_QKV_BIAS);
@@ -792,6 +842,7 @@
 #pragma unroll
             for (int i = 0; i < RB; i++) {
                 if (WQ8) acc[i] = dot16q(wv[j][i], reinterpret_cast<const float4(&)[4]>(xr[j]), acc[i]);
+                else if (WP) acc[i] = dot8h(wv[j][i], sd[(j * RB + i) >> 2], (j * RB + i) & 3, xr[j][0], xr[j][1], acc[i]);
                 else acc[i] = dot8(wv[j][i], xr[j][0], xr[j][XPC - 1], acc[i]);
             }
         if (first_group) {
@@ -811,7 +862,8 @@
         {
             const bool more = g < ngroups;
             gemv_rows<EPI, RB>(more ? g : 0, rows);
-            gemv_load<RB, KQ>(more ? wrs : wnone, rowbytes, rows, voff, wv);
+            if (WP) gemv_load_side<SW>(more ? srs : snone, tid * (SW * 4), (more ? g : 0) * (256 * SW * 4), sd);
+            gemv_load<RB, KQ, WP>(more ? wrs : wnone, rowbytes, rows, voff, wv);
             if (LOGIT && WQ8 && wave == 0) {
 #pragma unroll
                 for (int i = 0; i < RB; i++) wsc[i] = a.wscale[rows[i]];
@@ -2842,6 +2894,8 @@
     return 2;
 }
 
+int gemv_rowgroup(int rows) { return gemv_rb(rows); }
+
 VOX_KB_KNOB(g_gemv_maxb, 0);
 int gemv_grid(int rows) {
     const int ng = rows / gemv_rb(rows), maxb = g_gemv_maxb ? g_gemv_maxb : GEMV_MAX_BLOCKS;
@@ -2872,7 +2926,7 @@
 
 template <int P, int E, int RB, int Q8>
 static hipError_t gemv_k(const GemvArgs& a, int grid, hipStream_t st) {
-    const int kq = ((Q8 ? a.K >> 4 : a.K >> 3) + 255) / 256;
+    const int kq = ((Q8 == WF_Q8 ? a.K >> 4 : a.K >> 3) + 255) / 256;
     switch (kq) {
 #define KQ_CASE(Q) case Q: hipLaunchKernelGGL((k_gemv<P, E, RB, Q, Q8>), dim3(grid), dim3(256), 0, st, a); break;
         KQ_CASE(1) KQ_CASE(2) KQ_CASE(3) KQ_CASE(4) KQ_CASE(5)
@@ -2883,24 +2937,43 @@
     return hipSuccess;
 }
 
+template <int P, int E>
+constexpr bool gemv_p13 = (P == PRO_NONE && (E == EPI_STORE || E == EPI_RESID)) || (P == PRO_NORM && E == EPI_QKV) ||
+                          (P == PRO_NORM_ADA && E == EPI_SWIGLU) ||
+                          (P == PRO_NORM && (E == EPI_LOGITS || E == EPI_LOGITS_ALT));
+
+template <int P, int E, int RB>
+static hipError_t gemv_q(const GemvArgs& a, int grid, hipStream_t st) {
+    if (a.wscale) return gemv_k<P, E, RB, WF_Q8>(a, grid, st);
+    if constexpr (gemv_p13<P, E>) {
+        if (a.wp_main) return gemv_k<P, E, RB, WF_P13>(a, grid, st);
+    } else if (a.wp_main) {
+        return hipErrorInvalidValue;
+    }
+    return gemv_k<P, E, RB, WF_BF16>(a, grid, st);
+}
+template <int P, int E, int RB>
+static const void* gemv_fn_q(const GemvArgs& a, int kq) {
+    if (a.wscale) return gemv_fn<P, E, RB, WF_Q8>(kq);
+    if constexpr (gemv_p13<P, E>) {
+        if (a.wp_main) return gemv_fn<P, E, RB, WF_P13>(kq);
+    } else if (a.wp_main) {
+        return nullptr;
+    }
+    return gemv_fn<P, E, RB, WF_BF16>(kq);
+}
+
 const void* gemv_kernel(int pro, int epi, const GemvArgs& a) {
     const int rb = gemv_rb(a.rows);
     const int kq = ((a.wscale ? a.K >> 4 : a.K >> 3) + 255) / 256;
-#define GEMV_FN(P, E)                                                                     \
-    if (pro == P && epi == E)                                                             \
-        return rb == 8 ? (a.wscale ? gemv_fn<P, E, 8, 1>(kq) : gemv_fn<P, E, 8, 0>(kq))   \
-             : rb == 2 ? (a.wscale ? gemv_fn<P, E, 2, 1>(kq) : gemv_fn<P, E, 2, 0>(kq))   \
-                       : (a.wscale ? gemv_fn<P, E, 4, 1>(kq) : gemv_fn<P, E, 4, 0>(kq));
+#define GEMV_FN(P, E)         \
+    if (pro == P && epi == E) \
+        return rb == 8 ? gemv_fn_q<P, E, 8>(a, kq) : rb == 2 ? gemv_fn_q<P, E, 2>(a, kq) : gemv_fn_q<P, E, 4>(a, kq);
     GEMV_FN(PRO_NONE, EPI_STORE) GEMV_FN(PRO_NONE, EPI_RESID) GEMV_FN(PRO_NORM, EPI_QKV)
     GEMV_FN(PRO_NORM_ADA, EPI_SWIGLU) GEMV_FN(PRO_NORM, EPI_LOGITS) GEMV_FN(PRO_NORM, EPI_LOGITS_ALT)
     GEMV_FN(PRO_NORM, EPI_QKV_BIAS) GEMV_FN(PRO_NORM, EPI_SWIGLU)
 #undef GEMV_FN
     return nullptr;
-}
-
-template <int P, int E, int RB>
-static hipError_t gemv_q(const GemvArgs& a, int grid, hipStream_t st) {
-    return a.wscale ? gemv_k<P, E, RB, 1>(a, grid, st) : gemv_k<P, E, RB, 0>(a, grid, st);
 }
 
 hipError_t launch_gemv_timed(int pro, int epi, const GemvArgs& a, hipEvent_t start, hipEvent_t stop,
diff --git a/voxtral.c_amd/csrc/vox_synth.c b/voxtral.c_amd/csrc/vox_synth.c
--- a/voxtral.c_amd/csrc/vox_synth.c
+++ b/voxtral.c_amd/csrc/vox_synth.c
@@ -2,6 +2,8 @@
 #include <stddef.h>
 #include <stdint.h>
 #include <string.h>
+
+#include "vox_wpack.h"
 
 static inline uint64_t splitmix64(uint64_t x) {
     x += 0x9E3779B97F4A7C15ull;
@@ -80,3 +82,17 @@
     for (long long r = 0; r < rows; r++)
         for (long long c = 0; c < cols; c++) out[r * cols + c] = (float)q[r * cols + c] * scales[r];
 }
+
+int vox_wpack13_scan(const uint16_t *w, size_t n, int *emin, int *emax, int *D) {
+    return vox_wpack13_scan_(w, n, emin, emax, D);
+}
+void vox_wpack13_pack(const uint16_t *w, long long rows, long long K, int D, uint32_t *main, uint8_t *side) {
+    vox_wpack13_pack_(w, rows, K, D, main, side);
+}
+void vox_wpack13_unpack(const uint32_t *main, const uint8_t *side, long long rows, long long K, int D, uint16_t *w) {
+    vox_wpack13_unpack_(main, side, rows, K, D, w);
+}
+int vox_wpack13_side_words_of(long long K, int rb) { return vox_wpack13_side_words(K, rb); }
+void vox_wpack13_side_layout(const uint8_t *side, long long rows, long long K, int rb, int swiglu, uint32_t *out) {
+    vox_wpack13_side_layout_(side, rows, K, rb, swiglu, out);
+}
diff --git a/voxtral.c_amd/csrc/vox_wpack.h b/voxtral.c_amd/csrc/vox_wpack.h
--- /dev/null
+++ b/voxtral.c_amd/csrc/vox_wpack.h
@@ -0,0 +1,122 @@
+#ifndef VOX_WPACK_H
+#define VOX_WPACK_H
+#include <stddef.h>
+#include <stdint.h>
+#include <string.h>
+
+#define VOX_WPACK_MAX_SPAN 29
+#define VOX_WPACK_MAX_D 40
+
+static inline void vox_wpack13_scan_range(const uint16_t *w, size_t n, int *lo, int *hi, int *bad) {
+    int l = *lo, h = *hi, b = *bad;
+    for (size_t i = 0; i < n; i++) {
+        const int e = (w[i] >> 7) & 0xff, m = w[i] & 0x7f;
+        if (e == 0xff || (e == 0 && m)) b = 1;
+        if (e == 0) continue;
+        if (e < l) l = e;
+        if (e > h) h = e;
+    }
+    *lo = l;
+    *hi = h;
+    *bad = b;
+}
+static inline int vox_wpack13_choose(int lo, int hi, int bad, int *D) {
+    *D = 0;
+    if (bad || hi - lo > VOX_WPACK_MAX_SPAN) return 0;
+    if (hi < 0) return 1;
+    const int dlo = hi - 142, dhi = lo - 113;
+    const int d = dlo > 0 ? dlo : (dhi < 0 ? dhi : 0);
+    *D = d;
+    return d >= -VOX_WPACK_MAX_D && d <= VOX_WPACK_MAX_D;
+}
+static inline int vox_wpack13_scan_(const uint16_t *w, size_t n, int *emin, int *emax, int *D) {
+    int lo = 256, hi = -1, bad = 0;
+    vox_wpack13_scan_range(w, n, &lo, &hi, &bad);
+    *emin = hi < 0 ? 0 : lo;
+    *emax = hi < 0 ? 0 : hi;
+    return vox_wpack13_choose(lo, hi, bad, D);
+}
+
+static inline uint32_t vox_wpack13_code(uint16_t b, int D) {
+    const uint32_t s = b >> 15, e = (b >> 7) & 0xff, m = b & 0x7f;
+    if (e == 0) return s << 12;
+    return s << 12 | (uint32_t)((int)e - 112 - D) << 7 | m;
+}
+static inline uint16_t vox_wpack13_decode(uint32_t code, int D) {
+    const uint32_t s = code >> 12 & 1, e5 = code >> 7 & 0x1f, m = code & 0x7f;
+    if (e5 == 0) return (uint16_t)(s << 15);
+    return (uint16_t)(s << 15 | (uint32_t)((int)e5 + 112 + D) << 7 | m);
+}
+
+static inline void vox_wpack13_pack8(const uint16_t *w, int D, uint32_t *main3, uint8_t *side) {
+    uint32_t c[8];
+    for (int k = 0; k < 8; k++) c[k] = vox_wpack13_code(w[k], D);
+    for (int p = 0; p < 3; p++)
+        main3[p] = c[2 * p] << 3 | c[2 * p + 1] << 19 | ((c[6] >> (3 * p)) & 7) | ((c[7] >> (3 * p)) & 7) << 16;
+    *side = (uint8_t)(c[6] >> 9 | (c[7] >> 9) << 4);
+}
+static inline void vox_wpack13_unpack8(const uint32_t *main3, uint8_t side, int D, uint16_t *w) {
+    uint32_t c6 = (uint32_t)(side & 15) << 9, c7 = (uint32_t)(side >> 4) << 9;
+    for (int p = 0; p < 3; p++) {
+        w[2 * p] = vox_wpack13_decode(main3[p] >> 3 & 0x1fff, D);
+        w[2 * p + 1] = vox_wpack13_decode(main3[p] >> 19, D);
+        c6 |= (main3[p] & 7) << (3 * p);
+        c7 |= (main3[p] >> 16 & 7) << (3 * p);
+    }
+    w[6] = vox_wpack13_decode(c6, D);
+    w[7] = vox_wpack13_decode(c7, D);
+}
+
+static inline void vox_wpack13_pack_rows(const uint16_t *w, long long r0, long long r1, long long K, int D,
+                                         uint32_t *main, uint8_t *side) {
+    const long long kc = K / 8;
+    for (long long r = r0; r < r1; r++)
+        for (long long c = 0; c < kc; c++)
+            vox_wpack13_pack8(w + r * K + c * 8, D, main + (r * kc + c) * 3, side + r * kc + c);
+}
+static inline void vox_wpack13_pack_(const uint16_t *w, long long rows, long long K, int D, uint32_t *main,
+                                     uint8_t *side) {
+#pragma omp parallel for schedule(static) num_threads(16)
+    for (long long r = 0; r < rows; r++) vox_wpack13_pack_rows(w, r, r + 1, K, D, main, side);
+}
+static inline void vox_wpack13_unpack_(const uint32_t *main, const uint8_t *side, long long rows, long long K, int D,
+                                       uint16_t *w) {
+    const long long kc = K / 8;
+#pragma omp parallel for schedule(static) num_threads(16)
+    for (long long r = 0; r < rows; r++)
+        for (long long c = 0; c < kc; c++)
+            vox_wpack13_unpack8(main + (r * kc + c) * 3, side[r * kc + c], D, w + r * K + c * 8);
+}
+
+static inline long long vox_wpack13_row(long long g, int i, int rb, int swiglu) {
+    if (!swiglu) return g * rb + i;
+    const long long u = g * (rb / 2) + (i >> 1);
+    return ((u >> 4) << 5) + (u & 15) + ((i & 1) << 4);
+}
+static inline int vox_wpack13_kq(long long K) { return (int)((K / 8 + 255) / 256); }
+static inline int vox_wpack13_side_words(long long K, int rb) { return (vox_wpack13_kq(K) * rb + 3) / 4; }
+
+static inline void vox_wpack13_side_groups(const uint8_t *side, long long g0, long long g1, long long K, int rb,
+                                           int swiglu, uint32_t *out) {
+    const long long kc = K / 8;
+    const int kq = vox_wpack13_kq(K), sw = vox_wpack13_side_words(K, rb);
+    for (long long g = g0; g < g1; g++)
+        for (int t = 0; t < 256; t++) {
+            uint32_t *rec = out + (g * 256 + t) * sw;
+            memset(rec, 0, (size_t)sw * 4);
+            for (int j = 0; j < kq; j++)
+                for (int i = 0; i < rb; i++) {
+                    const int s = j * rb + i, q = s & 3;
+                    long long c = (long long)(j * 4 + t / 64) * 64 + t % 64;
+                    if (c >= kc) c = 0;
+                    const uint32_t b = side[vox_wpack13_row(g, i, rb, swiglu) * kc + c];
+                    rec[s >> 2] |= (b & 15) << (12 - 4 * q) | (b >> 4) << (28 - 4 * q);
+                }
+        }
+}
+static inline void vox_wpack13_side_layout_(const uint8_t *side, long long rows, long long K, int rb, int swiglu,
+                                            uint32_t *out) {
+#pragma omp parallel for schedule(static) num_threads(16)
+    for (long long g = 0; g < rows / rb; g++) vox_wpack13_side_groups(side, g, g + 1, K, rb, swiglu, out);
+}
+#endif
diff --git a/voxtral.c_amd/vox_hip.py b/voxtral.c_amd/vox_hip.py
--- a/voxtral.c_amd/vox_hip.py
+++ b/voxtral.c_amd/vox_hip.py
@@ -20,11 +20,31 @@
 ConfigC = config_struct_class()
 WeightsC = weights_struct_class()
 
+class WPackStatsC(ctypes.Structure):
+    _fields_ = [("packed_tensors", ctypes.c_int), ("raw_tensors", ctypes.c_int),
+                ("packed_bytes", ctypes.c_longlong), ("packed_raw_bytes", ctypes.c_longlong),
+                ("raw_bytes", ctypes.c_longlong), ("pack_ms", ctypes.c_double)]
+
+
+def gemv_wpack(W_bf16, x, packed: bool):
+    init()
+    W = np.ascontiguousarray(W_bf16, np.uint16)
+    xv = np.ascontiguousarray(x, np.float32)
+    rows, K = W.shape
+    assert xv.shape == (K,)
+    y = np.empty(rows, np.float32)
+    rc = lib().vox_hip_gemv_wpack(rows, K, W.ctypes.data, fptr(xv), fptr(y), int(packed))
+    if rc < 0:
+        _err("gemv_wpack")
+    return y, bool(rc)
+
+
 EXPORTS = [
     "vox_hip_init", "vox_hip_available", "vox_hip_shutdown", "vox_hip_memory_used",
     "vox_hip_last_error", "vox_hip_clear_error", "vox_hip_set_device", "vox_hip_config_voxtral_4b",
     "vox_hip_model_create", "vox_hip_model_free", "vox_hip_model_set_delay",
     "vox_hip_model_ada_scale", "vox_hip_model_set_kv_fp16", "vox_hip_stream_kv_fp16",
+    "vox_hip_model_wpack_stats", "vox_hip_gemv_wpack",
     "vox_hip_set_gemm_planes", "vox_hip_gemm_planes", "vox_hip_set_gemmf_wait",
     "vox_hip_stream_create", "vox_hip_stream_free",
     "vox_hip_stream_reset", "vox_hip_stream_reset_decoder", "vox_hip_stream_encode_mel",
@@ -64,6 +84,8 @@
         "vox_hip_model_create": (P, [P, P, I]), "vox_hip_model_free": (None, [P]),
         "vox_hip_model_set_delay": (I, [P, I]), "vox_hip_model_ada_scale": (I, [P, fp]),
         "vox_hip_model_set_kv_fp16": (I, [P, I]), "vox_hip_stream_kv_fp16": (I, [P]),
+        "vox_hip_model_wpack_stats": (I, [P, P]),
+        "vox_hip_gemv_wpack": (I, [I, I, P, fp, fp, I]),
         "vox_hip_set_gemm_planes": (I, [I]), "vox_hip_gemm_planes": (I, []),
         "vox_hip_set_gemmf_wait": (I, [I]),
         "vox_hip_stream_create": (P, [P]), "vox_hip_stream_free": (None, [P]),
@@ -164,6 +186,12 @@
         if lib().vox_hip_model_set_kv_fp16(self.h, int(on)) != 0:
             _err("set_kv_fp16")
 
+    def wpack_stats(self) -> dict:
+        st = WPackStatsC()
+        if lib().vox_hip_model_wpack_stats(self.h, ctypes.byref(st)) != 0:
+            _err("wpack_stats")
+        return {name: getattr(st, name) for name, _ in WPackStatsC._fields_}
+
     def ada_scale(self):
         c = self.cfg
         out = np.empty(c.dec_layers * c.dec_dim, np.float32)
```

After: 740.8, median of 6. 1.09x the previous value.
